# mcan1999/vulkan-raytracing

Hardware: AMD Instinct MI355X
Metric: Mrays/sec (primary+secondary) at 1920×1080 depth 4; 1/2/4/8-GPU scaling (higher is better)
Workload: dtype f32

## Files before the change

include/rt_api.h:

```cpp
#ifndef RT_API_H
#define RT_API_H

#include <stddef.h>
#include <stdint.h>

#ifdef __cplusplus
extern "C" {
#endif

typedef struct rt_ctx rt_ctx;

enum rt_status {
  RT_OK = 0,
  RT_ERR_INVALID_ARGUMENT = 1,
  RT_ERR_NOT_READY = 2,
  RT_ERR_DEVICE = 3,
  RT_ERR_OUT_OF_MEMORY = 4,
  RT_ERR_NO_DEVICE = 5
};

typedef struct rt_mesh_range {
  uint64_t first_float;
  uint64_t first_index;
  uint32_t prim_count;
// ... 86 lines not shown
#define RT_MATERIAL_TYPE_OF_INSTANCE 0xFFFFFFFFu
int rt_set_materials(rt_ctx* ctx, const rt_material* table, int n_materials, const uint32_t* prim_material, size_t n_prims);
int rt_set_instance_types(rt_ctx* ctx, const uint32_t* types, int n);

int rt_set_uniforms(rt_ctx* ctx, const rt_uniforms* u);

int rt_set_skybox(rt_ctx* ctx, const uint8_t* const faces_rgba8[6], int w, int h);

int rt_trace(rt_ctx* ctx, int width, int height, float* out_rgba32f_host, rt_stats* stats);

int rt_trace_shard(rt_ctx* ctx, int width, int height, int band_rows, int shard, int n_shards,
                   void* d_out, size_t out_capacity_bytes, void* hip_stream);
int rt_set_batch(rt_ctx* ctx, int n_frames, const rt_instance* instances, int n, const rt_uniforms* uniforms, int update);
int rt_trace_shard_batch(rt_ctx* ctx, int width, int height, int band_rows, int shard, int n_shards,
                         void* d_out, size_t frame_stride_bytes, size_t out_capacity_bytes, void* hip_stream);
int rt_trace_async(rt_ctx* ctx, int width, int height);
int rt_trace_wait(rt_ctx* ctx, const void** pixels, rt_stats* stats);

int rt_assemble_shards(rt_ctx* ctx, const void* d_gathered, int n_shards, size_t shard_stride_bytes, int width, int height,
                       int band_rows, void* d_frame, size_t frame_capacity_bytes, void* hip_stream);

int rt_shard_rows(int height, int band_rows, int shard, int n_shards);

int rt_synchronize(rt_ctx* ctx);
int rt_get_stats(rt_ctx* ctx, rt_stats* stats);
int rt_set_timing(rt_ctx* ctx, int enabled);

int rt_set_param(rt_ctx* ctx, const char* name, int value);

int rt_intersect(rt_ctx* ctx, size_t n, const float* rays8_host, int any_hit, rt_hit* out_host, int counting,
                 rt_stats* stats);

typedef struct rt_hit_attr {
  float position[3];
  int32_t object_index;
  float normal[3];
  uint32_t reserved;
} rt_hit_attr;

int rt_intersect_device(rt_ctx* ctx, size_t n, const void* d_rays8, int any_hit, void* d_hits, void* d_attr, void* hip_stream);

#define RT_RAY_FLAG_OPAQUE                 0x001u
#define RT_RAY_FLAG_NO_OPAQUE              0x002u
#define RT_RAY_FLAG_TERMINATE_ON_FIRST_HIT 0x004u
#define RT_RAY_FLAG_SKIP_CLOSEST_HIT       0x008u
#define RT_RAY_FLAG_CULL_BACK_FACING       0x010u
#define RT_RAY_FLAG_CULL_FRONT_FACING      0x020u
#define RT_RAY_FLAG_CULL_OPAQUE            0x040u
#define RT_RAY_FLAG_CULL_NO_OPAQUE         0x080u
#define RT_RAY_FLAG_SKIP_TRIANGLES         0x100u
#define RT_RAY_FLAG_SKIP_AABBS             0x200u
#define RT_INSTANCE_FLAG_FACING_CULL_DISABLE 0x1u
#define RT_INSTANCE_FLAG_FLIP_FACING         0x2u
#define RT_INSTANCE_FLAG_FORCE_OPAQUE        0x4u
#define RT_INSTANCE_FLAG_FORCE_NO_OPAQUE     0x8u
#define RT_HIT_KIND_FRONT_FACING 0xFEu
#define RT_HIT_KIND_BACK_FACING  0xFFu

int rt_intersect_device_flags(rt_ctx* ctx, size_t n, const void* d_rays8, const void* d_ray_words, uint32_t ray_flags, uint32_t cull_mask, void* d_hits, void* d_attr, void* hip_stream);

int rt_intersect_device_hits(rt_ctx* ctx, size_t n, const void* d_rays8, const void* d_ray_words, uint32_t ray_flags, uint32_t cull_mask,
                             uint32_t max_hits, void* d_hits, void* d_attr, void* d_counts, void* hip_stream);

int rt_closest_point_device(rt_ctx* ctx, size_t n, const void* d_points4, uint32_t cull_mask, void* d_hits, void* d_attr, void* hip_stream);
int rt_closest_point(rt_ctx* ctx, size_t n, const float* points4_host, uint32_t cull_mask, rt_hit* out_host, int counting, rt_stats* stats);

#define RT_OVERLAP_ANY 0x1u
int rt_overlap_boxes_device(rt_ctx* ctx, size_t n, const void* d_boxes8, uint32_t cull_mask, uint32_t flags,
                            uint32_t max_ids, void* d_ids, void* d_counts, void* hip_stream);
int rt_overlap_boxes(rt_ctx* ctx, size_t n, const float* boxes8_host, uint32_t cull_mask, uint32_t flags,
                     uint32_t max_ids, int32_t* ids_host, uint32_t* counts_host, int counting, rt_stats* stats);

int rt_sweep_spheres_device(rt_ctx* ctx, size_t n, const void* d_sweeps8, uint32_t cull_mask,
                            void* d_hits, void* d_attr, void* hip_stream);
int rt_sweep_spheres(rt_ctx* ctx, size_t n, const float* sweeps8_host, uint32_t cull_mask,
                     rt_hit* out_host, int counting, rt_stats* stats);

int rt_shade_rays_device(rt_ctx* ctx, size_t n_points, uint32_t n_samples, const void* d_rays8, void* d_sample_rgba, void* d_point_rgba, void* hip_stream);

int rt_trace_counting(rt_ctx* ctx, int width, int height, float* out_rgba32f_host, rt_stats* stats);

int rt_debug_check_builders(const float* verts6, size_t n_floats, const uint32_t* idx, size_t n_idx, uint64_t* out8);
int rt_debug_sizing(int n_cu, int resident_per_cu, int trace_blocks, uint32_t ovf_stride, uint64_t* out2);

const char* rt_last_error(const rt_ctx* ctx);
const char* rt_device_info(const rt_ctx* ctx);
int rt_abi_version(void);

#ifdef __cplusplus
}
#endif
#endif
```

vulkan_raytracing_amd/api.py:

```python
import ctypes as C

import numpy as np

from . import _native

HIT_DTYPE = np.dtype([("t", np.float32), ("u", np.float32), ("v", np.float32), ("prim", np.int32), ("inst", np.int32)])
MESH_RANGE_DTYPE = np.dtype([("first_float", np.uint64), ("first_index", np.uint64), ("prim_count", np.uint32), ("reserved", np.uint32)])
INSTANCE_DTYPE = np.dtype([("transform", np.float32, 12), ("custom_index_and_mask", np.uint32), ("sbt_offset_and_flags", np.uint32), ("mesh", np.uint64)])
UNIFORMS_DTYPE = np.dtype([("position", np.float32, 4), ("right", np.float32, 4), ("up", np.float32, 4), ("forward", np.float32, 4),
                           ("light_position", np.float32, 3), ("light_intensity", np.float32),
                           ("max_bounce_count", np.uint32), ("samples_per_pixel", np.uint32),
                           ("center_object_type", np.uint32), ("orbiting_object_type", np.uint32),
                           ("orbiting_object_primitive_offset", np.uint32), ("orbiting_object_vertex_offset", np.uint32)])
MATERIAL_DTYPE = np.dtype([("ka", np.float32, 3), ("ns", np.float32), ("kd", np.float32, 3), ("ni", np.float32), ("ks", np.float32, 3), ("type", np.uint32)])
MATERIAL_TYPE_OF_INSTANCE = 0xFFFFFFFF
assert MATERIAL_DTYPE.itemsize == 48
assert INSTANCE_DTYPE.itemsize == 64 and UNIFORMS_DTYPE.itemsize == 104 and MESH_RANGE_DTYPE.itemsize == 24


class RtStats(C.Structure):
    _fields_ = [("rays_primary", C.c_uint64), ("rays_secondary", C.c_uint64), ("rays_shadow", C.c_uint64),
                ("node_visits", C.c_uint64), ("tri_tests", C.c_uint64), ("node_visits_shadow", C.c_uint64), ("tri_tests_shadow", C.c_uint64),
                ("diag", C.c_uint64 * 6), ("closest_rays", C.c_uint64),
                ("ms_frame", C.c_float), ("ms_raygen", C.c_float), ("ms_trace_closest", C.c_float), ("ms_trace_shadow", C.c_float),
                ("ms_shade", C.c_float), ("ms_resolve", C.c_float),
                ("launches_trace_closest", C.c_uint32), ("launches_total", C.c_uint32), ("timed_frames", C.c_uint32), ("ms_tail", C.c_float),
                ("bvh_node_bytes", C.c_uint32), ("bvh_tri_bytes", C.c_uint32), ("tail_faults", C.c_uint32), ("frames_rerendered", C.c_uint32),
                ("blob_tiles", C.c_uint64), ("blob_tiles_large", C.c_uint64), ("blob_tiles_refused", C.c_uint64), ("blob_nodes", C.c_uint64), ("blob_tris", C.c_uint64),
                ("tile_rays", C.c_uint64), ("tile_rays_handed_on", C.c_uint64), ("tile_diag", C.c_uint64 * 6), ("rays_shadow_untraced", C.c_uint64)]

    def as_dict(self):
        return {k: (list(getattr(self, k)) if k in ("diag", "tile_diag") else getattr(self, k)) for k, _ in self._fields_}

    @property
    def rays_total(self):
        return self.rays_primary + self.rays_secondary + self.rays_shadow


RAY_FLAG_NONE = 0x000
RAY_FLAG_OPAQUE = 0x001
RAY_FLAG_NO_OPAQUE = 0x002
RAY_FLAG_TERMINATE_ON_FIRST_HIT = 0x004
RAY_FLAG_SKIP_CLOSEST_HIT = 0x008
RAY_FLAG_CULL_BACK_FACING = 0x010
RAY_FLAG_CULL_FRONT_FACING = 0x020
RAY_FLAG_CULL_OPAQUE = 0x040
RAY_FLAG_CULL_NO_OPAQUE = 0x080
RAY_FLAG_SKIP_TRIANGLES = 0x100
RAY_FLAG_SKIP_AABBS = 0x200
INSTANCE_FLAG_FACING_CULL_DISABLE = 0x1
INSTANCE_FLAG_FLIP_FACING = 0x2
INSTANCE_FLAG_FORCE_OPAQUE = 0x4
INSTANCE_FLAG_FORCE_NO_OPAQUE = 0x8
HIT_KIND_FRONT_FACING = 0xFE
HIT_KIND_BACK_FACING = 0xFF
OVERLAP_ANY = 0x1

EXPORTS = ["rt_create", "rt_create_frame_slot", "rt_destroy", "rt_upload_geometry", "rt_build_blas", "rt_set_instances", "rt_set_instances_device", "rt_refit_blas_device", "rt_set_materials", "rt_set_instance_types", "rt_set_uniforms", "rt_set_skybox",
           "rt_trace", "rt_trace_async", "rt_trace_wait", "rt_trace_shard", "rt_set_batch", "rt_trace_shard_batch", "rt_assemble_shards", "rt_shard_rows", "rt_synchronize", "rt_get_stats", "rt_set_timing", "rt_intersect",
           "rt_trace_counting", "rt_intersect_device", "rt_intersect_device_flags", "rt_intersect_device_hits", "rt_closest_point_device", "rt_closest_point", "rt_overlap_boxes_device", "rt_overlap_boxes", "rt_sweep_spheres_device", "rt_sweep_spheres", "rt_shade_rays_device", "rt_set_param", "rt_debug_check_builders", "rt_debug_sizing", "rt_last_error", "rt_device_info", "rt_abi_version"]

_LIBS = {}


def lib(variant=None):
    if variant not in _LIBS:
        L = _native.load_rt(variant)
        vp = C.c_void_p
        L.rt_create.argtypes = [C.POINTER(vp), C.c_int]
        L.rt_create_frame_slot.argtypes = [vp, C.POINTER(vp)]
        L.rt_destroy.argtypes = [vp]
        L.rt_destroy.restype = None
        L.rt_upload_geometry.argtypes = [vp, vp, C.c_size_t, vp, C.c_size_t, vp, C.c_int]
        L.rt_build_blas.argtypes = [vp, C.c_int]
        L.rt_set_instances.argtypes = [vp, vp, C.c_int, C.c_int]
        L.rt_set_instances_device.argtypes = [vp, vp, C.c_int, C.c_int, vp]
        L.rt_refit_blas_device.argtypes = [vp, C.c_int, vp, C.c_size_t, vp]
        L.rt_set_materials.argtypes = [vp, vp, C.c_int, vp, C.c_size_t]
        L.rt_set_instance_types.argtypes = [vp, vp, C.c_int]
        L.rt_set_uniforms.argtypes = [vp, vp]
        L.rt_set_skybox.argtypes = [vp, C.POINTER(vp), C.c_int, C.c_int]
        L.rt_trace.argtypes = [vp, C.c_int, C.c_int, vp, C.POINTER(RtStats)]
        L.rt_trace_counting.argtypes = [vp, C.c_int, C.c_int, vp, C.POINTER(RtStats)]
        L.rt_trace_async.argtypes = [vp, C.c_int, C.c_int]
        L.rt_trace_wait.argtypes = [vp, C.POINTER(vp), C.POINTER(RtStats)]
        L.rt_trace_shard.argtypes = [vp, C.c_int, C.c_int, C.c_int, C.c_int, C.c_int, vp, C.c_size_t, vp]
        L.rt_trace_shard_batch.argtypes = [vp, C.c_int, C.c_int, C.c_int, C.c_int, C.c_int, vp, C.c_size_t, C.c_size_t, vp]
        L.rt_set_batch.argtypes = [vp, C.c_int, vp, C.c_int, vp, C.c_int]
        L.rt_assemble_shards.argtypes = [vp, vp, C.c_int, C.c_size_t, C.c_int, C.c_int, C.c_int, vp, C.c_size_t, vp]
        L.rt_shard_rows.argtypes = [C.c_int] * 4
        L.rt_synchronize.argtypes = [vp]
        L.rt_get_stats.argtypes = [vp, C.POINTER(RtStats)]
        L.rt_set_timing.argtypes = [vp, C.c_int]
        L.rt_set_param.argtypes = [vp, C.c_char_p, C.c_int]
        L.rt_debug_check_builders.argtypes = [vp, C.c_size_t, vp, C.c_size_t, vp]
        L.rt_debug_sizing.argtypes = [C.c_int, C.c_int, C.c_int, C.c_uint32, vp]
        L.rt_intersect.argtypes = [vp, C.c_size_t, vp, C.c_int, vp, C.c_int, C.POINTER(RtStats)]
        L.rt_intersect_device.argtypes = [vp, C.c_size_t, vp, C.c_int, vp, vp, vp]
        L.rt_intersect_device_flags.argtypes = [vp, C.c_size_t, vp, vp, C.c_uint32, C.c_uint32, vp, vp, vp]
        L.rt_intersect_device_hits.argtypes = [vp, C.c_size_t, vp, vp, C.c_uint32, C.c_uint32, C.c_uint32, vp, vp, vp, vp]
        L.rt_closest_point_device.argtypes = [vp, C.c_size_t, vp, C.c_uint32, vp, vp, vp]
        L.rt_closest_point.argtypes = [vp, C.c_size_t, vp, C.c_uint32, vp, C.c_int, C.POINTER(RtStats)]
        L.rt_sweep_spheres_device.argtypes = [vp, C.c_size_t, vp, C.c_uint32, vp, vp, vp]
        L.rt_sweep_spheres.argtypes = [vp, C.c_size_t, vp, C.c_uint32, vp, C.c_int, C.POINTER(RtStats)]
        L.rt_overlap_boxes_device.argtypes = [vp, C.c_size_t, vp, C.c_uint32, C.c_uint32, C.c_uint32, vp, vp, vp]
        L.rt_overlap_boxes.argtypes = [vp, C.c_size_t, vp, C.c_uint32, C.c_uint32, C.c_uint32, vp, vp, C.c_int, C.POINTER(RtStats)]
        L.rt_shade_rays_device.argtypes = [vp, C.c_size_t, C.c_uint32, vp, vp, vp, vp]
        L.rt_last_error.argtypes = [vp]
        L.rt_last_error.restype = C.c_char_p
        L.rt_device_info.argtypes = [vp]
        L.rt_device_info.restype = C.c_char_p
        _LIBS[variant] = L
    return _LIBS[variant]


class RtError(RuntimeError):

    def __init__(self, code, fn, detail):
        super().__init__("RT API exception: return code %d (%s): %s" % (code, fn, detail))
        self.code = code


def _p(a):
    return a.ctypes.data_as(C.c_void_p)


class RtContext:

    def __init__(self, device=0, _parent=None, variant=None):
        self.L = _parent.L if _parent is not None else lib(variant)
        h = C.c_void_p()
        if _parent is not None:
            rc = self.L.rt_create_frame_slot(_parent.h, C.byref(h))
        else:
            rc = self.L.rt_create(C.byref(h), device)
        if rc:
            raise RtError(rc, "rt_create_frame_slot" if _parent is not None else "rt_create", self.L.rt_last_error(None).decode())
        self.h = h
        self.device = _parent.device if _parent is not None else device

    def frame_slot(self):
        return RtContext(_parent=self)

    def _chk(self, rc, fn):
        if rc:
            raise RtError(rc, fn, self.L.rt_last_error(self.h).decode())

    def close(self):
        if getattr(self, "h", None):
            self.L.rt_destroy(self.h)
            self.h = None

    def __del__(self):
        try:
            self.close()
        except Exception:
            pass

    @property
    def device_info(self):
        return self.L.rt_device_info(self.h).decode()

    def upload_geometry(self, verts6, idx, ranges, build=True):
        verts6 = np.ascontiguousarray(verts6, np.float32)
        idx = np.ascontiguousarray(idx, np.uint32)
        r = np.zeros(len(ranges), MESH_RANGE_DTYPE)
        for i, (ff, fi, pc) in enumerate(ranges):
            r[i] = (ff, fi, pc, 0)
        self._chk(self.L.rt_upload_geometry(self.h, _p(verts6), verts6.size, _p(idx), idx.size, _p(r), len(ranges)), "rt_upload_geometry")
        if build:
            for m in range(len(ranges)):
                self.build_blas(m)

    def build_blas(self, mesh):
        self._chk(self.L.rt_build_blas(self.h, mesh), "rt_build_blas")

    def set_instances(self, instances, update=False):
        inst = np.ascontiguousarray(instances, INSTANCE_DTYPE)
        self._chk(self.L.rt_set_instances(self.h, _p(inst), len(inst), int(update)), "rt_set_instances")
# ... 436 lines not shown
```

vulkan_raytracing_amd/csrc/kernels.hip:

```cpp
#include <hip/hip_runtime.h>

#include "rt_kernels.h"

namespace rt {

struct F3 { float x, y, z; };
__device__ __forceinline__ F3 mk3(float x, float y, float z) { F3 r; r.x = x; r.y = y; r.z = z; return r; }
__device__ __forceinline__ F3 add3(F3 a, F3 b) { return mk3(a.x + b.x, a.y + b.y, a.z + b.z); }
__device__ __forceinline__ F3 sub3(F3 a, F3 b) { return mk3(a.x - b.x, a.y - b.y, a.z - b.z); }
__device__ __forceinline__ F3 mul3(F3 a, float s) { return mk3(a.x * s, a.y * s, a.z * s); }
__device__ __forceinline__ F3 neg3(F3 a) { return mk3(-a.x, -a.y, -a.z); }
__device__ __forceinline__ float dot3(F3 a, F3 b) { return __builtin_fmaf(a.z, b.z, __builtin_fmaf(a.y, b.y, a.x * b.x)); }
__device__ __forceinline__ F3 cross3(F3 a, F3 b) {
  return mk3(__builtin_fmaf(a.y, b.z, -(a.z * b.y)), __builtin_fmaf(a.z, b.x, -(a.x * b.z)), __builtin_fmaf(a.x, b.y, -(a.y * b.x)));
}
__device__ __forceinline__ float length3(F3 v) { return __builtin_sqrtf(dot3(v, v)); }
__device__ __forceinline__ F3 normalize3(F3 v) { float inv = 1.0f / length3(v); return mul3(v, inv); }
__device__ __forceinline__ F3 fma3(float s, F3 a, F3 b) { return mk3(__builtin_fmaf(s, a.x, b.x), __builtin_fmaf(s, a.y, b.y), __builtin_fmaf(s, a.z, b.z)); }
__device__ __forceinline__ F3 reflect3(F3 I, F3 N) { float k = 2.0f * dot3(N, I); return fma3(-k, N, I); }

__device__ __forceinline__ F3 xform_point(const float* m, F3 p) {
  return mk3(__builtin_fmaf(m[2], p.z, __builtin_fmaf(m[1], p.y, m[0] * p.x)) + m[3],
             __builtin_fmaf(m[6], p.z, __builtin_fmaf(m[5], p.y, m[4] * p.x)) + m[7],
             __builtin_fmaf(m[10], p.z, __builtin_fmaf(m[9], p.y, m[8] * p.x)) + m[11]);
// ... 741 lines not shown
        for (uint32_t w = 0; w < blockDim.y; w++) { const float4 c = s_col[w][lane]; r += c.x; g += c.y; b += c.z; al += c.w; }
        const float nn = (float)spp;
        const uint32_t p = ly * (uint32_t)f.width + x;
        store_pixel(f, fi * f.out_frame_stride + p, make_float4(r / nn, g / nn, b / nn, al / nn));
        st_stream(&f.sample_color[fi * spp * npx1 + p], make_float4(0.f, 0.f, 0.f, PIXEL_DONE));
      }
    } else if (missed) st_stream(&f.sample_color[sid], miss_col);
  }
  if (survive || run_tile) {
    const uint32_t v = shard * f.shard_cap + slot;
    if (!f.pixel_runs) {
      const F3 o = f.batch_k > 1 ? mk3(bt.position[fi][0], bt.position[fi][1], bt.position[fi][2]) : mk3(u.position[0], u.position[1], u.position[2]);
      st_stream(&f.ray_o[0][v], make_float4(o.x, o.y, o.z, f.entry != nullptr ? __uint_as_float(tile) : 10000.0f));
    }
    st_stream(&f.ray_d[0][v], survive ? make_float4(d.x, d.y, d.z, __uint_as_float(sid)) : make_float4(0.f, 0.f, 0.f, __uint_as_float(SID_DEAD)));
  }
}

struct TraceArgs {
  SceneDev sc;
  const float4* ray_o;
  const float4* ray_d;
  const uint32_t* tails;
  uint32_t* work;
  uint32_t shard_cap;
  float4* hit_a;
  int32_t* hit_inst;
  const float4* sh_c;
  float4* sample_color;
  HitRec* raw_out;
  int32_t* ovf_stack;
  uint32_t* counters;
  union {
    float tmin;
    uint32_t query_word;
  };
  uint32_t rays_per_lane;
  uint32_t min_blocks;
  const EntryRec* entry;
  union {
    const uint32_t* sh_e;
    const uint32_t* ray_words;
  };
};

constexpr int MODE_CLOSEST = 0;
constexpr int MODE_SHADOW = 1;
constexpr int MODE_QUERY = 3;
constexpr int MODE_QUERY_FLAGS = 4;


#ifndef RT_REFILL_MIN
#define RT_REFILL_MIN 16
#endif
#ifndef RT_KEEP_NUM
#define RT_KEEP_NUM 5
#endif
#ifndef RT_INTERIOR_UNROLL
#define RT_INTERIOR_UNROLL 2
#endif
#ifndef RT_WIDE_UNROLL
#define RT_WIDE_UNROLL 1
#endif
#ifndef RT_WAVES_PER_EU
#define RT_WAVES_PER_EU 5
#endif
#ifndef RT_LEAF_CHAIN
#define RT_LEAF_CHAIN 1
#endif
#ifndef RT_STACK2_LDS
#define RT_STACK2_LDS 12
#endif
constexpr int STACK2_LDS = RT_STACK2_LDS;
constexpr uint32_t REFILL_MIN = RT_REFILL_MIN;

#ifdef RT_EXP_PHASE_SEL
#define PH_BEGIN(k) uint64_t ph_b##k = 0; if (COUNT && RT_EXP_PHASE_SEL == k) ph_b##k = __builtin_readcyclecounter();
#define PH_END(k) if (COUNT && RT_EXP_PHASE_SEL == k && lane == 0) { diag_iters++; diag_busy += __builtin_readcyclecounter() - ph_b##k; }
#else
#define PH_BEGIN(k)
#define PH_END(k)
#endif

template <int MODE, bool ANY, bool COUNT, bool WIDE, bool ENTRY = false, bool FAR = true, bool CONT = false>
__device__ __forceinline__ void trace_body(const TraceArgs& a) {
  constexpr bool RAYS8 = MODE == MODE_QUERY || MODE == MODE_QUERY_FLAGS;
  constexpr bool QF = MODE == MODE_QUERY_FLAGS;
  __shared__ int s_stack[4][STACK2_LDS + 1][64];
  __shared__ float4 s_rays[4][2][64];
  __shared__ float4 s_out[4][64];
  __shared__ int2 s_outq[4][64];
  __shared__ uint32_t s_ent[((ENTRY && MODE == MODE_SHADOW) || QF) ? 4 : 1][64];
  __shared__ float4 s_inst[LDS_INSTANCES ? LDS_INSTANCES : 1][5];
  {
    uint32_t total = 0;
#pragma unroll
    for (int t = 0; t < N_SHARDS; t++) total += ld_cursor(a.tails + t * CNT_STRIDE);
    uint32_t want = (total + 256u * a.rays_per_lane - 1u) / (256u * a.rays_per_lane);
    want = (want + (N_SHARDS - 1)) & ~(uint32_t)(N_SHARDS - 1);
    if (want < a.min_blocks) want = a.min_blocks;
    if (blockIdx.x >= want) return;
  }
  const int n_lds_inst = a.sc.n_inst < LDS_INSTANCES ? a.sc.n_inst : LDS_INSTANCES;
  if ((int)threadIdx.x < n_lds_inst) {
    const InstanceDev* I = a.sc.inst + threadIdx.x;
    const float4* mp = reinterpret_cast<const float4*>(I->w2o);
    s_inst[threadIdx.x][0] = mp[0]; s_inst[threadIdx.x][1] = mp[1]; s_inst[threadIdx.x][2] = mp[2];
    s_inst[threadIdx.x][3] = make_float4(I->q_lo[0], I->q_lo[1], I->q_lo[2], __int_as_float(I->blas_root));
    s_inst[threadIdx.x][4] = make_float4(I->q_scale[0], I->q_scale[1], I->q_scale[2], __uint_as_float(I->mask));
  }
  __syncthreads();
  const uint32_t lane = threadIdx.x & 63u, wave = threadIdx.x >> 6;
  int* const stk = &s_stack[wave][0][lane];
  int32_t* const ovf = a.ovf_stack + (size_t)(blockIdx.x * 256u + threadIdx.x) * a.sc.ovf_stride;
  uint64_t cnt_nodes = 0, cnt_tris = 0, diag_iters = 0, diag_busy = 0;
  const uint64_t diag_t0 = COUNT ? __builtin_readcyclecounter() : 0;

  uint32_t shard = blockIdx.x & (N_SHARDS - 1), tried = 0;
  uint32_t pf_base = 0, pf_count = 0;
  float4 pf_o = make_float4(0, 0, 0, 0), pf_d = pf_o;
  uint32_t pf_e = ENTRY_FROM_ROOT;
  uint32_t chunk_base = 0, chunk_count = 0, chunk_pos = 0;
  auto prefetch = [&]() {
    pf_count = 0;
    while (tried < (uint32_t)N_SHARDS) {
      const uint32_t size = ld_cursor(a.tails + shard * CNT_STRIDE);
      uint32_t off = 0;
      if (lane == 0 && size) off = atomicAdd(a.work + shard * CNT_STRIDE, 64u);
      off = (uint32_t)__builtin_amdgcn_readfirstlane((int)off);
      if (size && off < size) { pf_base = shard * a.shard_cap + off; pf_count = (size - off) < 64u ? (size - off) : 64u; break; }
      shard = (shard + 1u) & (N_SHARDS - 1); tried++;
    }
    if (lane < pf_count) {
      if constexpr (RAYS8) {
        const size_t r = 2u * (size_t)(pf_base + lane);
        pf_o = ld_stream(&a.ray_o[r]); pf_d = ld_stream(&a.ray_o[r + 1u]);
        if (QF) {
          const uint32_t w = a.ray_words ? (uint32_t)ld_stream(reinterpret_cast<const int*>(a.ray_words) + pf_base + lane) : 0xFF000000u;
          pf_e = ((a.query_word | w) & QF_FLAGS) | (a.query_word & w & 0xFF000000u);
        }
      } else {
        pf_o = ld_stream(&a.ray_o[pf_base + lane]); pf_d = ld_stream(&a.ray_d[pf_base + lane]);
      }
      if (ENTRY && MODE == MODE_SHADOW) pf_e = (uint32_t)ld_stream(reinterpret_cast<const int*>(a.sh_e) + pf_base + lane);
    }
  };
  auto promote = [&]() {
    s_rays[wave][0][lane] = pf_o; s_rays[wave][1][lane] = pf_d;
    if ((ENTRY && MODE == MODE_SHADOW) || QF) s_ent[wave][lane] = pf_e;
    chunk_base = pf_base; chunk_count = pf_count; chunk_pos = 0;
    prefetch();
  };
  prefetch();
  promote();

  uint32_t out_count = 0;
  auto flush = [&]() {
    if (lane < out_count) {
      const float4 r = s_out[wave][lane];
      const int2 k = s_outq[wave][lane];
      if (MODE == MODE_CLOSEST) { st_stream(&a.hit_a[k.x], r); st_stream(&a.hit_inst[k.x], k.y); }
      else if (MODE == MODE_SHADOW) {
        float cr = 0.08f, cg = 0.24f, cb = 0.08f;
        if (r.x != 0.0f || a.sc.n_materials != 0) {
          const float4 shc = ld_stream(&a.sh_c[(uint32_t)k.y]);
          if (r.x != 0.0f) { cr = shc.x; cg = shc.y; cb = shc.z; }
          else { const F3 amb = ambient_of(a.sc, __float_as_uint(shc.w)); cr = amb.x; cg = amb.y; cb = amb.z; }
        }
        st_stream(&a.sample_color[(uint32_t)k.x], make_float4(cr, cg, cb, 1.0f));
      }
      else { HitRec h; h.t = r.x; h.u = r.y; h.v = r.z; h.prim = (int)__float_as_uint(r.w); h.inst = k.y; a.raw_out[k.x] = h; }
    }
    out_count = 0;
  };

  bool need = true;
  uint32_t q = 0, sid = 0;
  float tmin_ray = 0.f, tmax = 0.f;
  uint32_t qword = 0;
  F3 wo = mk3(0, 0, 0), wd = mk3(0, 0, 1), co = wo, cd = wd, qs = mk3(1, 1, 1), qb = mk3(0, 0, 0);
  uint3 rot = make_uint3(0u, 0u, 0u);
  bool far = false;
  float best_t = 0.f, best_u = 0.f, best_v = 0.f;
  int best_prim = -1, best_inst = -1, cur_inst = -1, sp = 0, cur = REF_DONE;
  const char* const node_bytes = WIDE ? reinterpret_cast<const char*>(a.sc.wide_nodes) : reinterpret_cast<const char*>(a.sc.blas_nodes);

  auto push = [&](int v) {
    if (sp < STACK2_LDS) stk[sp * 64] = v;
    else *reinterpret_cast<volatile int32_t*>(ovf + (sp - STACK2_LDS)) = v;
    sp++;
  };
  auto pop = [&]() {
    sp--;
    if (sp < STACK2_LDS) cur = stk[sp * 64];
    else cur = *reinterpret_cast<volatile int32_t*>(ovf + (sp - STACK2_LDS));
  };

  auto to_instance = [&](int ii, int& root, uint32_t& imask) {
    float4 m0, m1, m2, ql, qsc;
    if (ii < n_lds_inst) { m0 = s_inst[ii][0]; m1 = s_inst[ii][1]; m2 = s_inst[ii][2]; ql = s_inst[ii][3]; qsc = s_inst[ii][4]; }
    else {
      const InstanceDev* I = a.sc.inst + ii;
      const float4* mp = reinterpret_cast<const float4*>(I->w2o);
      m0 = mp[0]; m1 = mp[1]; m2 = mp[2];
      ql = make_float4(I->q_lo[0], I->q_lo[1], I->q_lo[2], __int_as_float(I->blas_root));
      qsc = make_float4(I->q_scale[0], I->q_scale[1], I->q_scale[2], __uint_as_float(I->mask));
    }
    root = __float_as_int(ql.w); imask = __float_as_uint(qsc.w);
    if ((imask & 0xFFu) != 0u) {
      float m[12];
      m[0] = m0.x; m[1] = m0.y; m[2] = m0.z; m[3] = m0.w; m[4] = m1.x; m[5] = m1.y; m[6] = m1.z; m[7] = m1.w;
      m[8] = m2.x; m[9] = m2.y; m[10] = m2.z; m[11] = m2.w;
      co = xform_point(m, wo); cd = xform_vec(m, wd);
      const float qlo3[3] = {ql.x, ql.y, ql.z}, qsc3[3] = {qsc.x, qsc.y, qsc.z};
      quant_space(co, cd, qlo3, qsc3, qs, qb, rot); far = FAR && quant_far_o(co, qlo3, qsc3);
    }
  };

  for (;;) {
    PH_BEGIN(5)
    const uint64_t need_mask = __ballot(need);
    const uint32_t n_need = (uint32_t)__builtin_popcountll(need_mask);
    if (n_need >= REFILL_MIN || n_need == 64u) {
      if (chunk_pos == chunk_count && pf_count > 0) promote();
      if (chunk_pos < chunk_count) {
        const uint32_t rank = prefix_rank(need_mask);
        const uint32_t avail = chunk_count - chunk_pos;
        if (need && rank < avail) {
          const uint32_t ci = chunk_pos + rank;
          q = chunk_base + ci;
          const float4 ro = s_rays[wave][0][ci], rd = s_rays[wave][1][ci];
          if (RAYS8) { tmin_ray = ro.w; tmax = rd.w; }
          else { tmax = ro.w; sid = __float_as_uint(rd.w); }
          if (QF) qword = s_ent[wave][ci];
          wo = mk3(ro.x, ro.y, ro.z); wd = mk3(rd.x, rd.y, rd.z);
          co = wo; cd = wd;
          cur_inst = -1;
          stk[0] = REF_DONE;
          bool handed_on = false;
          if (CONT && (__float_as_uint(ro.w) & CONT_FLAG) != 0u) {
            handed_on = true;
            const uint32_t ent = __float_as_uint(ro.w);
            const uint32_t tile = ent & 0xFFFFFFu, mask = (ent >> 24) & 15u;
            const int4* rp = reinterpret_cast<const int4*>(a.entry + tile);
            const int4 r0 = rp[0], r1 = rp[1];
            const uint32_t n_rest = (((uint32_t)r0.x >> 4) & 15u) - 1u;
            const int wk[4] = {r0.z, r0.w, r1.x, r1.y};
            sp = 1;
#pragma unroll
            for (uint32_t k = 0; k < 4u; k++)
              if (k < n_rest && ((mask >> (n_rest - 1u - k)) & 1u) != 0u) { stk[sp * 64] = wk[k]; sp++; }
            sp--; cur = stk[sp * 64];
            quant_space(co, cd, a.sc.tlas_q_lo, a.sc.tlas_q_scale, qs, qb, rot); far = false;
            const float4 inc = a.hit_a[q];
            best_t = inc.x; best_u = inc.y; best_v = inc.z; best_prim = (int)__float_as_uint(inc.w); best_inst = a.hit_inst[q];
          } else
          if (ENTRY) {
            uint32_t ent;
            if (MODE == MODE_SHADOW) ent = s_ent[wave][ci];
            else ent = __float_as_uint(ro.w);
            const bool rev_flag = MODE == MODE_SHADOW && (ent & ENTRY_REVERSE) != 0u;
            if (MODE == MODE_SHADOW) ent &= ~ENTRY_REVERSE;
            int4 r0 = make_int4((int)ENTRY_EMPTY, REF_DONE, 0, 0), r1 = make_int4(0, 0, 0, 0);
            if (ent != ENTRY_FROM_ROOT) {
              const int4* rp = reinterpret_cast<const int4*>(a.entry + ent);
              r0 = rp[0]; r1 = rp[1];
            }
            const uint32_t hdr = (uint32_t)r0.x;
            if (ent == ENTRY_FROM_ROOT) {
              quant_space(co, cd, a.sc.tlas_q_lo, a.sc.tlas_q_scale, qs, qb, rot); far = FAR && quant_far_o(co, a.sc.tlas_q_lo, a.sc.tlas_q_scale);
              sp = 1; cur = a.sc.tlas_root + (a.sc.batch_samples ? (int)frame_of(sid, a.sc.batch_samples) * a.sc.tlas_stride : 0);
            } else if (hdr == ENTRY_EMPTY) {
              sp = 1; cur = REF_DONE;
            } else {
              const uint32_t nw = hdr & 15u, n_rm = (hdr >> 4) & 15u, ia = hdr >> 8;
              const bool rev = MODE == MODE_SHADOW && rev_flag && nw > n_rm;
              int cur_new = r0.y;
              const int wk[6] = {r0.z, r0.w, r1.x, r1.y, r1.z, r1.w};
#pragma unroll
              for (uint32_t k = 0; k < 6u; k++)
                if (k < nw) {
                  if (rev && k == n_rm) cur_new = wk[k];
                  else stk[((!rev || k < n_rm) ? 1u + k : 1u + nw + n_rm - k) * 64u] = wk[k];
                }
              if (rev) stk[(1u + n_rm) * 64u] = r0.y;
              sp = 1 + (int)nw;
              cur = cur_new;
              __builtin_amdgcn_sched_barrier(0);
              if (ia != ENTRY_NO_INST) { int root; uint32_t imask; to_instance((int)ia, root, imask); cur_inst = (int)ia; }
              else { quant_space(co, cd, a.sc.tlas_q_lo, a.sc.tlas_q_scale, qs, qb, rot); far = FAR && quant_far_o(co, a.sc.tlas_q_lo, a.sc.tlas_q_scale); }
            }
          } else {
            quant_space(co, cd, a.sc.tlas_q_lo, a.sc.tlas_q_scale, qs, qb, rot); far = FAR && quant_far_o(co, a.sc.tlas_q_lo, a.sc.tlas_q_scale);
            sp = 1;
            cur = a.sc.tlas_root;
            if (!RAYS8 && a.sc.batch_samples) cur += (int)frame_of(sid, a.sc.batch_samples) * a.sc.tlas_stride;
          }
          if (!(CONT && handed_on)) { best_t = (ENTRY && MODE == MODE_CLOSEST) ? 10000.0f : tmax; best_u = 0.f; best_v = 0.f; best_prim = -1; best_inst = -1; }
          need = false;
        }
        chunk_pos += n_need < avail ? n_need : avail;
      } else if (n_need == 64u) { flush(); break; }
    }
    PH_END(5)
    const uint32_t live = 64u - (uint32_t)__builtin_popcountll(__ballot(need));
    const uint32_t keep_going = (live * RT_KEEP_NUM + 7u) >> 3;

    auto interior_step = [&]() {
      if (WIDE) {
        if (cur >= 0) {
          const uint4* np = reinterpret_cast<const uint4*>(node_bytes + ((uint32_t)cur << 6));
          const uint4 X = np[0], Y = np[1], Z = np[2], R = np[3];
          if (COUNT) cnt_nodes++;
// ... 314 lines not shown
          const F3 spec = mk3((Iv * ks.x) * sp, (Iv * ks.y) * sp, (Iv * ks.z) * sp);
          const F3 amb = ambient_of(a.sc, mat);
          sh_c = fma3(w, add3(diff, spec), amb); sh_w = __uint_as_float(mat);
          nd = L; sh_tmax = dist;
          push_shadow = true;
          if (f.settle_dead_shadow_rays && __float_as_uint(sh_c.x) == __float_as_uint(amb.x) && __float_as_uint(sh_c.y) == __float_as_uint(amb.y) &&
              __float_as_uint(sh_c.z) == __float_as_uint(amb.z)) {
            st_stream(&f.sample_color[sid], make_float4(amb.x, amb.y, amb.z, 1.0f));
            push_shadow = false; settled = true;
          }
          if (f.light_entry != nullptr) {
            const F3 v = sub3(no, light);
            const float ax = __builtin_fabsf(v.x), ay = __builtin_fabsf(v.y), az = __builtin_fabsf(v.z);
            const int axis = (ax >= ay && ax >= az) ? 0 : (ay >= az ? 1 : 2);
            const float vc = axis == 0 ? v.x : (axis == 1 ? v.y : v.z), va = axis == 0 ? v.y : (axis == 1 ? v.z : v.x), vb = axis == 0 ? v.z : (axis == 1 ? v.x : v.y);
            const float c = __builtin_fabsf(vc);
            if (c > 0.0f) {
              const float T8 = (float)(8 * f.light_tiles);
              const float px = (va / c + 1.0f) * 0.5f * T8, py = (1.0f - vb / c) * 0.5f * T8;
              const int tx = min(max((int)(px * 0.125f), 0), f.light_tiles - 1), ty = min(max((int)(py * 0.125f), 0), f.light_tiles - 1);
              const int face = 2 * axis + (vc < 0.0f ? 1 : 0);
              sh_ent = (uint32_t)((face * f.light_tiles + ty) * f.light_tiles + tx) | (NdotL < 0.0f ? ENTRY_REVERSE : 0u);
            }
          }
        }
      } else if (type == 1u) {
        no = fma3(0.01f, N, P);
        nd = reflect3(d, N);
        push_next = true;
      } else if (type == 2u) {
        float ndoti = dot3(d, N);
        const bool outwards = ndoti > 0.0f;
        if (outwards) { N = neg3(N); ndoti = -ndoti; }
        const float ratio = M ? (outwards ? M->ni : 1.0f / M->ni) : (outwards ? 1.52f : (1.0f / 1.52f));
        const float k = 1.0f - (ratio * ratio) * (1.0f - ndoti * ndoti);
        if (k < 0.0f) { nd = reflect3(d, N); no = fma3(0.01f, N, P); }
        else {
          const float c = __builtin_fmaf(ratio, ndoti, __builtin_sqrtf(k));
          nd = normalize3(fma3(-c, N, mul3(d, ratio)));
          no = fma3(-0.01f, N, P);
        }
        push_next = true;
      } else {
        if (bounce == 0 && f.pixel_runs) {
          no = mk3(U.position[0], U.position[1], U.position[2]);
          if constexpr (BATCH) { const uint32_t fk = frame_of(sid, a.sc.batch_samples); no = mk3(a.bt.position[fk][0], a.bt.position[fk][1], a.bt.position[fk][2]); }
        } else {
          const float4 ro = ld_stream(&f.ray_o[cur][q]);
          no = mk3(ro.x, ro.y, ro.z);
        }
        nd = d; push_next = true;
      }
      if (push_next && last) {
        push_next = false;
        st_stream(&f.sample_color[sid], ambient_default<REG>());
      }
    }
  }
  {
    const uint64_t m_st = __ballot(settled);
    if (lane == 0 && m_st != 0ull) {
      __hip_atomic_fetch_add(f.counters + cnt_tail(Q_SHADOW0, (int)shard), (uint32_t)__builtin_popcountll(m_st), __ATOMIC_RELAXED, __HIP_MEMORY_SCOPE_AGENT);
      __hip_atomic_fetch_add(f.counters + cnt_work(Q_DEAD, (int)shard), (uint32_t)__builtin_popcountll(m_st), __ATOMIC_RELAXED, __HIP_MEMORY_SCOPE_AGENT);
    }
  }
  const uint32_t slot_n = wave_alloc(push_next, f.counters + cnt_tail(bounce + 1, (int)shard));
  if (push_next) {
    const uint32_t v = shard * f.shard_cap + slot_n;
    st_stream(&f.ray_o[nxt][v], make_float4(no.x, no.y, no.z, 10000.0f));
    st_stream(&f.ray_d[nxt][v], make_float4(nd.x, nd.y, nd.z, __uint_as_float(sid)));
  }
  if constexpr (RUNS) {
    if (in_range) {
      if (push_shadow) {
        st_stream(&f.sh_o[q], make_float4(no.x, no.y, no.z, sh_tmax));
        st_stream(&f.sh_c[q], make_float4(sh_c.x, sh_c.y, sh_c.z, sh_w));
        if (f.sh_e != nullptr) f.sh_e[q] = sh_ent;
      }
      st_stream(&f.sh_d[q], push_shadow ? make_float4(nd.x, nd.y, nd.z, __uint_as_float(sid)) : make_float4(0.f, 0.f, 0.f, __uint_as_float(SID_DEAD)));
    }
    const uint64_t m_sh = __ballot(push_shadow);
    if (lane == 0 && m_sh != 0ull) __hip_atomic_fetch_add(f.counters + cnt_tail(Q_SHADOW0, (int)shard), (uint32_t)__builtin_popcountll(m_sh), __ATOMIC_RELAXED, __HIP_MEMORY_SCOPE_AGENT);
  } else {
    const uint32_t slot_s = wave_alloc(push_shadow, f.counters + cnt_tail(Q_SHADOW, (int)shard));
    if (push_shadow) {
      const uint32_t v = f.sh_base + shard * f.shard_cap + slot_s;
      st_stream(&f.sh_o[v], make_float4(no.x, no.y, no.z, sh_tmax));
      st_stream(&f.sh_d[v], make_float4(nd.x, nd.y, nd.z, __uint_as_float(sid)));
      st_stream(&f.sh_c[v], make_float4(sh_c.x, sh_c.y, sh_c.z, sh_w));
      if (f.sh_e != nullptr) f.sh_e[v] = sh_ent;
    }
  }
}

template <bool TILE = false, bool BATCH = false, bool RUNS = false>
__device__ __forceinline__ void shade_body(const ShadeArgs& a, const int bounce) {
  const FrameDev& f = a.f;
  const UniformsDev& U = a.u;
  const uint32_t lane = threadIdx.x & 63u, wave = threadIdx.x >> 6;
  const int n_pass = TILE ? 2 : 1;
  for (int pass = 0; pass < n_pass; pass++) {
  uint32_t cnt[N_SHARDS], maxb = 0;
#pragma unroll
  for (int t = 0; t < N_SHARDS; t++) {
    if (TILE && pass) {
      uint32_t blobs = 0;
#pragma unroll
      for (int k = 0; k < BLOB_CLASSES; k++) blobs += ld_cursor(f.counters + cnt_tail(Q_BLOB_LIST + k, t));
      cnt[t] = blobs * (256u * ((U.samples_per_pixel + 3u) / 4u));
    } else cnt[t] = ld_cursor(f.counters + cnt_tail(bounce, t));
    maxb = max(maxb, (cnt[t] + 63u) >> 6);
  }
  const uint32_t n_waves = gridDim.x * 4u;
  for (uint32_t g = blockIdx.x * 4u + wave; g < maxb * N_SHARDS; g += n_waves) {
    const uint32_t shard = g & (N_SHARDS - 1), base = (g >> 3) << 6;
    uint32_t n = 0;
#pragma unroll
    for (int t = 0; t < N_SHARDS; t++) n = (shard == (uint32_t)t) ? cnt[t] : n;
    if (base >= n) continue;
    const uint32_t q = shard * f.shard_cap + ((TILE && pass) ? f.shard_cap - n : 0u) + base + lane;
    shade_slot<TILE, BATCH, RUNS, false>(a, bounce, shard, q, base + lane < n, HIT_DEAD, make_float4(0.f, 0.f, 0.f, 0.f));
  }
  }
}

template <bool TILE, bool BATCH, bool RUNS = false>
__global__ __launch_bounds__(256) void k_shade(ShadeArgs a) { shade_body<TILE, BATCH, RUNS>(a, a.bounce); }

#include "kernels_beam.inc"

struct TailArgs {
  TraceArgs tr;
  ShadeArgs sh;
  uint32_t first_bounce;
  uint32_t* barrier;
  uint32_t* fault;
};

__device__ __forceinline__ void grid_barrier(uint32_t* bar, uint32_t* fault, uint32_t& phase) {
  __syncthreads();
  phase++;
  if (threadIdx.x == 0) {
    __threadfence();
    const uint32_t target = phase * gridDim.x;
    __hip_atomic_fetch_add(bar, 1u, __ATOMIC_RELAXED, __HIP_MEMORY_SCOPE_AGENT);
    uint32_t spins = 0;
    while (__hip_atomic_load(bar, __ATOMIC_RELAXED, __HIP_MEMORY_SCOPE_AGENT) < target) {
      __builtin_amdgcn_s_sleep(8);
      if (++spins > (1u << 24)) { __hip_atomic_store(fault, 1u, __ATOMIC_RELAXED, __HIP_MEMORY_SCOPE_AGENT); break; }
    }
    __threadfence();
  }
  __syncthreads();
}

template <bool COUNT, bool WIDE, bool BATCH = false>
__global__ __launch_bounds__(256) void k_tail(TailArgs t) {
  uint32_t phase = 0;
  const uint32_t max_bounce = t.sh.u.max_bounce_count;
  for (uint32_t b = t.first_bounce; b <= max_bounce; b++) {
    uint32_t live = 0;
#pragma unroll
    for (int k = 0; k < N_SHARDS; k++) live += ld_cursor(t.tr.counters + cnt_tail((int)b, k));
    if (live == 0 || ld_cursor(t.fault) != 0u) break;
    TraceArgs a = t.tr;
    a.ray_o = t.sh.f.ray_o[b & 1u]; a.ray_d = t.sh.f.ray_d[b & 1u];
    a.tails = t.tr.counters + cnt_tail((int)b, 0);
    a.work = t.tr.counters + cnt_work((int)b, 0);
    trace_body<MODE_CLOSEST, false, COUNT, WIDE>(a);
    grid_barrier(t.barrier, t.fault, phase);
    if (ld_cursor(t.fault) != 0u) return;
    shade_body<false, BATCH>(t.sh, (int)b);
    grid_barrier(t.barrier, t.fault, phase);
    if (ld_cursor(t.fault) != 0u) return;
  }
}

__global__ __launch_bounds__(256) void k_resolve(FrameDev f, UniformsDev u) {
  const uint32_t npx1 = (uint32_t)(f.rows * f.width);
  const uint32_t lane = threadIdx.x & 63u, wave = (uint32_t)__builtin_amdgcn_readfirstlane((int)(threadIdx.x >> 6));
  const uint32_t tile_rows1 = ((uint32_t)f.rows + 7u) >> 3;
  const uint32_t trow = blockIdx.y * 4u + wave;
  if (trow < tile_rows1 * (uint32_t)f.batch_k) {
    const uint32_t fi = f.batch_k > 1 ? trow / tile_rows1 : 0u, by = trow - fi * tile_rows1;
    const uint32_t x = blockIdx.x * 8u + (lane & 7u), ly = by * 8u + (lane >> 3);
    if (!tile_is_sky(f, fi, blockIdx.x, by, trow * gridDim.x + blockIdx.x) && x < (uint32_t)f.width && ly < (uint32_t)f.rows) {
      const uint32_t p1 = ly * (uint32_t)f.width + x;
      const size_t s0 = (size_t)fi * u.samples_per_pixel * npx1 + p1;
      if (f.sample_color[s0].w != PIXEL_DONE) {
        float r = 0.f, g = 0.f, b = 0.f, al = 0.f;
        for (uint32_t i = 0; i < u.samples_per_pixel; i++) {
          const float4 c = ld_stream(&f.sample_color[s0 + (size_t)i * npx1]);
          r += c.x; g += c.y; b += c.z; al += c.w;
        }
        const float nn = (float)u.samples_per_pixel;
        store_pixel(f, fi * f.out_frame_stride + p1, make_float4(r / nn, g / nn, b / nn, al / nn));
      }
    }
  }
  const uint32_t p = (blockIdx.y * gridDim.x + blockIdx.x) * blockDim.x + threadIdx.x, n_threads = gridDim.x * gridDim.y * blockDim.x;
  if (f.counters_next)
    for (uint32_t i = p; i < (uint32_t)CNT_WORDS; i += n_threads) f.counters_next[i] = 0u;
  if (f.cover_next)
    for (uint32_t i = p; i < f.cover_words; i += n_threads) f.cover_next[i] = 0u;
  if (blockIdx.x == 0 && blockIdx.y == 0 && f.stats_out) {
    __shared__ unsigned long long s_q[N_QUEUES];
    const uint32_t t = threadIdx.x;
    if (t < (uint32_t)N_QUEUES) {
      unsigned long long n = 0;
      for (int k = 0; k < N_SHARDS; k++) n += ld_cursor(f.counters + cnt_tail((int)t, k));
      s_q[t] = n;
    }
    __syncthreads();
    if (f.hint && t >= 1u && t < (uint32_t)CNT_MAX_BOUNCES)
      __hip_atomic_store(f.hint + t, (uint32_t)(s_q[t] > 0xFFFFFFFFull ? 0xFFFFFFFFull : s_q[t]), __ATOMIC_RELAXED, __HIP_MEMORY_SCOPE_SYSTEM);
    auto cnt64 = [&](int word) { return (unsigned long long)ld_cursor(f.counters + word) | ((unsigned long long)ld_cursor(f.counters + word + 1) << 32); };
    if (t < (uint32_t)STAT_WORDS) {
      unsigned long long v = 0;
      if (t == STAT_QUEUE0) { v = s_q[0] + s_q[Q_TILE_RAYS] - s_q[Q_DEAD]; for (int k = 0; k < N_SHARDS; k++) v -= ld_cursor(f.counters + cnt_work(Q_TILE_RAYS, k)); }
      else if (t == STAT_TILE_RAYS) v = s_q[Q_TILE_RAYS];
      else if (t == STAT_CONT_RAYS) { for (int k = 0; k < N_SHARDS; k++) v += ld_cursor(f.counters + cnt_work(Q_TILE_RAYS, k)); }
      else if (t >= STAT_BLOB && t < STAT_BLOB + 5) v = ld_cursor(f.counters + CNT_BLOB_STATS + (int)(t - STAT_BLOB));
      else if (t >= STAT_TILE_DIAG && t < STAT_TILE_DIAG + 6) v = cnt64(CNT_TILE_DIAG + 2 * (int)(t - STAT_TILE_DIAG));
      else if (t == STAT_SECONDARY) { for (uint32_t b = 1; b <= u.max_bounce_count && b < (uint32_t)CNT_MAX_BOUNCES; b++) v += s_q[b]; }
      else if (t == STAT_SHADOW) v = s_q[Q_SHADOW] + s_q[Q_SHADOW0];
      else if (t == STAT_SHADOW_UNTRACED) { for (int k = 0; k < N_SHARDS; k++) v += ld_cursor(f.counters + cnt_work(Q_DEAD, k)); }
      else if (t == STAT_QUEUE1) v = s_q[1];
      else if (t == STAT_FAULT) v = ld_cursor(f.counters + CNT_FAULT);
      else if (t == STAT_FAULT_TOTAL) {
        uint32_t total = f.fault_total ? f.fault_total[0] : 0u;
        if (f.fault_total && ld_cursor(f.counters + CNT_FAULT) != 0u) { total++; f.fault_total[0] = total; }
        v = total;
      }
      else if (t == STAT_NODE_VISITS) v = cnt64(CNT_NODE_VISITS);
      else if (t == STAT_TRI_TESTS) v = cnt64(CNT_TRI_TESTS);
      else if (t == STAT_NODE_VISITS_SH) v = cnt64(CNT_NODE_VISITS_SH);
      else if (t == STAT_TRI_TESTS_SH) v = cnt64(CNT_TRI_TESTS_SH);
      else if (t >= STAT_DIAG && t < STAT_DIAG + 3) v = cnt64(CNT_DIAG + 2 * (int)(t - STAT_DIAG));
      else if (t >= STAT_DIAG + 3 && t < STAT_DIAG + 6) v = cnt64(CNT_DIAG_SH + 2 * (int)(t - STAT_DIAG - 3));
      __hip_atomic_store(f.stats_out + t, v, __ATOMIC_RELAXED, __HIP_MEMORY_SCOPE_SYSTEM);
    }
  }
}

int trace_threads_per_block() { return 256; }

static dim3 raygen_grid(int width, int rows, uint32_t spp, int batch_k, dim3& block) {
  const uint32_t wpb = spp < 4u ? spp : 4u;
  block = dim3(64, wpb);
  return dim3(((uint32_t)width + 7u) >> 3, (((uint32_t)rows + 7u) >> 3) * (uint32_t)batch_k, (spp + wpb - 1u) / wpb);
}
size_t raygen_block_count(int width, int rows, uint32_t spp, int batch_k) {
  dim3 b; const dim3 g = raygen_grid(width, rows, spp, batch_k, b);
  return (size_t)g.x * g.y * g.z;
}
void launch_raygen(const SceneDev& sc, const FrameDev& f, const UniformsDev& u, const BatchTab& bt, hipStream_t s) {
  dim3 b; const dim3 g = raygen_grid(f.width, f.rows, u.samples_per_pixel, f.batch_k, b);
  hipLaunchKernelGGL(k_raygen, g, b, 0, s, sc, f, u, bt);
}
size_t jitter_table_elems(int width, int rows, uint32_t spp) {
  return (size_t)(((uint32_t)width + 7u) >> 3) * (size_t)(((uint32_t)rows + 7u) >> 3) * spp * 64u;
}
void launch_jitter_table(const FrameDev& f, uint32_t spp, float2* table, hipStream_t s) {
  dim3 b; const dim3 g = raygen_grid(f.width, f.rows, spp, 1, b);
  hipLaunchKernelGGL(k_jitter_table, g, b, 0, s, f, spp, table);
}

void launch_cover(const SceneDev& sc, const CoverViews& a, uint32_t max_boxes_per_instance, uint32_t* mask_block, hipStream_t s) {
  if (a.n <= 0 || a.v[0].n_inst <= 0 || max_boxes_per_instance == 0) return;
  hipLaunchKernelGGL(k_cover, dim3((max_boxes_per_instance + 255u) / 256u, (unsigned)a.v[0].n_inst, (unsigned)a.n), dim3(256), 0, s, sc, a, mask_block);
}

static TraceArgs make_args(const SceneDev& sc, uint32_t* counters, int queue, uint32_t shard_cap, int32_t* ovf) {
  TraceArgs a{};
  a.sc = sc;
  a.tmin = 0.001f;
  a.counters = counters;
  a.tails = counters + cnt_tail(queue, 0);
  a.work = counters + cnt_work(queue, 0);
  a.shard_cap = shard_cap;
  a.ovf_stack = ovf;
  a.rays_per_lane = 4; a.min_blocks = 8;
  return a;
}

template <int MODE, bool ANY>
static void launch_trace(const TraceArgs& a_in, bool counting, const LaunchCfg& cfg, hipStream_t s) {
  TraceArgs a = a_in;
  a.rays_per_lane = (uint32_t)cfg.rays_per_lane; a.min_blocks = (uint32_t)cfg.min_blocks;
  const dim3 g(cfg.trace_blocks), b(256);
#ifdef RT_ALT_KERNELS
  if (cfg.variant == 2) {
    if (counting) hipLaunchKernelGGL((k_trace_count<MODE, ANY, true>), g, b, 0, s, a);
    else hipLaunchKernelGGL((k_trace<MODE, ANY, true>), g, b, 0, s, a);
    return;
  }
  if (cfg.variant == 1) {
    if (counting) hipLaunchKernelGGL((k_trace4<MODE, ANY, true>), g, b, 0, s, a);
    else hipLaunchKernelGGL((k_trace4<MODE, ANY, false>), g, b, 0, s, a);
    return;
  }
#endif
  if (counting) hipLaunchKernelGGL((k_trace_count<MODE, ANY, false>), g, b, 0, s, a);
  else if constexpr (MODE == MODE_QUERY) hipLaunchKernelGGL((k_trace<MODE, ANY, false, false, true>), g, b, 0, s, a);
  else if (cfg.far) hipLaunchKernelGGL((k_trace<MODE, ANY, false, false, true>), g, b, 0, s, a);
  else hipLaunchKernelGGL((k_trace<MODE, ANY, false, false, false>), g, b, 0, s, a);
}

// ... 246 lines not shown
    if (valid && tmax > 0.001f) {
      F3 qs, qb; uint3 rot;
      quant_space(o, d, sc.tlas_q_lo, sc.tlas_q_scale, qs, qb, rot);
      const bool far = quant_far(qs, qb);
      const uint4* rp = reinterpret_cast<const uint4*>(sc.blas_nodes + sc.tlas_root);
      const uint4 Q0 = rp[0], Q1 = rp[1];
      float tn;
      const bool h0 = far || slab_q(Q0.x, Q0.y, Q0.z, qs, qb, rot, 0.001f, tmax, tn);
      const bool h1 = (far || slab_q(Q0.w, Q1.x, Q1.y, qs, qb, rot, 0.001f, tmax, tn)) && Q1.w != Q1.z;
      const int c0 = (int)Q1.z, c1 = (int)Q1.w;
      survive = (h0 && c0 < 0) || (h1 && c1 < 0);
#pragma unroll
      for (int k = 0; k < 2; k++) {
        const int ch = k ? c1 : c0;
        if ((k ? h1 : h0) && ch >= 0 && !survive) {
          const uint4* np = reinterpret_cast<const uint4*>(sc.blas_nodes + ch);
          const uint4 N0 = np[0], N1 = np[1];
          survive = far || slab_q(N0.x, N0.y, N0.z, qs, qb, rot, 0.001f, tmax, tn) || slab_q(N0.w, N1.x, N1.y, qs, qb, rot, 0.001f, tmax, tn);
        }
      }
    }
    if (!survive) {
      float4 c = make_float4(0.f, 0.f, 0.f, 0.f);
      if (valid) { const F3 s = sample_sky(sc, mk3(d.x, d.y, -d.z)); c = make_float4(s.x, s.y, s.z, 1.0f); }
      st_stream(&f.sample_color[sid], c);
    }
  }
  __shared__ uint32_t s_run[5];
  const uint64_t smask = __ballot(survive);
  if (lane == 0) s_run[wave] = (uint32_t)__builtin_popcountll(smask);
  __syncthreads();
  const uint32_t shard = blockIdx.x & (N_SHARDS - 1);
  if (threadIdx.x == 0) {
    uint32_t tot = 0;
    for (uint32_t w = 0; w < 4u; w++) { const uint32_t c = s_run[w]; s_run[w] = tot; tot += c; }
    s_run[4] = tot ? atomicAdd(f.counters + cnt_tail(0, (int)shard), tot) : 0u;
  }
  __syncthreads();
  if (survive) {
    const uint32_t v = shard * f.shard_cap + s_run[4] + s_run[wave] + prefix_rank(smask);
    st_stream(&f.ray_o[0][v], make_float4(o.x, o.y, o.z, tmax));
    st_stream(&f.ray_d[0][v], make_float4(d.x, d.y, d.z, __uint_as_float(sid)));
  }
}

__global__ __launch_bounds__(256) void k_resolve_points(const float4* __restrict__ sample_color, float4* __restrict__ out, uint32_t n_points,
                                                        uint32_t n_samples) {
  const uint32_t p = blockIdx.x * 256u + threadIdx.x;
  if (p >= n_points) return;
  float r = 0.f, g = 0.f, b = 0.f, al = 0.f;
  for (uint32_t i = 0; i < n_samples; i++) {
    const float4 c = ld_stream(&sample_color[p + (size_t)i * n_points]);
    r += c.x; g += c.y; b += c.z; al += c.w;
  }
  const float nn = (float)n_samples;
  out[p] = make_float4(r / nn, g / nn, b / nn, al / nn);
}

uint32_t ray_ingest_block_count(uint32_t n) { return (n + 255u) / 256u; }
void launch_ray_ingest(const SceneDev& sc, const FrameDev& f, const float4* rays, uint32_t n, hipStream_t s) {
  hipLaunchKernelGGL(k_ray_ingest, dim3(ray_ingest_block_count(n)), dim3(256), 0, s, sc, f, rays, n);
}
void launch_resolve_points(const float4* sample_color, float4* out, uint32_t n_points, uint32_t n_samples, hipStream_t s) {
  hipLaunchKernelGGL(k_resolve_points, dim3((n_points + 255u) / 256u), dim3(256), 0, s, sample_color, out, n_points, n_samples);
}

#include "kernels_closest.inc"

#include "kernels_overlap.inc"

#include "kernels_sweep.inc"

int tail_blocks_per_cu() {
  int n = 1 << 30, v = 0;
  if (hipOccupancyMaxActiveBlocksPerMultiprocessor(&v, k_tail<false, false>, 256, 0) != hipSuccess) return 0;
  n = min(n, v);
  if (hipOccupancyMaxActiveBlocksPerMultiprocessor(&v, k_tail<true, false>, 256, 0) != hipSuccess) return 0;
  n = min(n, v);
#ifdef RT_ALT_KERNELS
  if (hipOccupancyMaxActiveBlocksPerMultiprocessor(&v, k_tail<false, true>, 256, 0) != hipSuccess) return 0;
  n = min(n, v);
  if (hipOccupancyMaxActiveBlocksPerMultiprocessor(&v, k_tail<true, true>, 256, 0) != hipSuccess) return 0;
  n = min(n, v);
#endif
  return n;
}

void launch_tail(const SceneDev& sc, const FrameDev& f, const UniformsDev& u, const BatchTab& bt, int first_bounce, bool counting, const LaunchCfg& cfg, int tail_blocks, hipStream_t s) {
  TailArgs t{};
  t.tr = make_args(sc, f.counters, first_bounce, f.shard_cap, f.ovf_stack);
  t.tr.hit_a = f.hit_a; t.tr.hit_inst = f.hit_inst;
  t.tr.rays_per_lane = 1u; t.tr.min_blocks = 8u;
  t.sh = ShadeArgs{sc, f, u, first_bounce, bt};
  t.first_bounce = (uint32_t)first_bounce;
  t.barrier = f.counters + CNT_BARRIER; t.fault = f.counters + CNT_FAULT;
  const dim3 g((unsigned)tail_blocks), b(256);
#ifdef RT_ALT_KERNELS
  if (cfg.variant == 2) {
    if (counting) hipLaunchKernelGGL((k_tail<true, true>), g, b, 0, s, t);
    else hipLaunchKernelGGL((k_tail<false, true>), g, b, 0, s, t);
    return;
  }
#endif
  if (f.batch_k > 1) {
    if (counting) hipLaunchKernelGGL((k_tail<true, false, true>), g, b, 0, s, t);
    else hipLaunchKernelGGL((k_tail<false, false, true>), g, b, 0, s, t);
    return;
  }
  if (counting) hipLaunchKernelGGL((k_tail<true, false>), g, b, 0, s, t);
  else hipLaunchKernelGGL((k_tail<false, false>), g, b, 0, s, t);
}

void launch_shade(const SceneDev& sc, const FrameDev& f, const UniformsDev& u, const BatchTab& bt, int bounce, const LaunchCfg& cfg, hipStream_t s) {
  ShadeArgs a{sc, f, u, bounce, bt};
  if (f.batch_k > 1) hipLaunchKernelGGL((k_shade<false, true>), dim3(cfg.shade_blocks), dim3(256), 0, s, a);
#ifdef RT_ALT_KERNELS
  else if (bounce == 0 && f.shadow_runs) hipLaunchKernelGGL((k_shade<false, false, true>), dim3(cfg.shade_blocks), dim3(256), 0, s, a);
  else if (bounce == 0 && f.tile_blob != nullptr) hipLaunchKernelGGL((k_shade<true, false>), dim3(cfg.shade_blocks), dim3(256), 0, s, a);
#endif
  else hipLaunchKernelGGL((k_shade<false, false>), dim3(cfg.shade_blocks), dim3(256), 0, s, a);
}

template <typename T>
__global__ __launch_bounds__(256) void k_assemble(const T* __restrict__ gathered, T* __restrict__ out, uint32_t width, uint32_t height,
                                                   uint32_t band_rows, uint32_t n_shards, size_t shard_stride) {
  const uint32_t x = blockIdx.x * blockDim.x + threadIdx.x, y = blockIdx.y;
  if (x >= width || y >= height) return;
  const uint32_t band = y / band_rows, within = y - band * band_rows;
  const uint32_t shard = band % n_shards, local = (band / n_shards) * band_rows + within;
  out[(size_t)y * width + x] = gathered[(size_t)shard * shard_stride + (size_t)local * width + x];
}

void launch_assemble(const void* gathered, void* out, int width, int height, int band_rows, int n_shards, size_t shard_stride_px, bool rgba8, hipStream_t s) {
  const dim3 g(((uint32_t)width + 255u) / 256u, (uint32_t)height), b(256);
  if (rgba8) hipLaunchKernelGGL((k_assemble<uint32_t>), g, b, 0, s, (const uint32_t*)gathered, (uint32_t*)out, (uint32_t)width, (uint32_t)height, (uint32_t)band_rows, (uint32_t)n_shards, shard_stride_px);
  else hipLaunchKernelGGL((k_assemble<float4>), g, b, 0, s, (const float4*)gathered, (float4*)out, (uint32_t)width, (uint32_t)height, (uint32_t)band_rows, (uint32_t)n_shards, shard_stride_px);
}

void launch_resolve(const FrameDev& f, const UniformsDev& u, hipStream_t s) {
  const uint32_t tile_rows = (((uint32_t)f.rows + 7u) >> 3) * (uint32_t)f.batch_k;
  hipLaunchKernelGGL(k_resolve, dim3(((uint32_t)f.width + 7u) >> 3, (tile_rows + 3u) / 4u), dim3(256), 0, s, f, u);
}

}
```

vulkan_raytracing_amd/csrc/rt_api.cpp:

```cpp
#include "../../include/rt_api.h"

#include <hip/hip_runtime.h>

#include <algorithm>
#include <cmath>
#include <cstdio>
#include <cstring>
#include <map>
#include <mutex>
#include <queue>
#include <string>
#include <vector>

#include "blas_refit.h"
#include "bvh_build.h"
#include "bvh_gpu.h"
#include "rt_device.h"
#include "rt_kernels.h"
#include "tlas_gpu.h"

using namespace rt;

static_assert(sizeof(rt_instance) == 64, "rt_instance must mirror VkAccelerationStructureInstanceKHR (64 B)");
static_assert(sizeof(rt_uniforms) == 104, "rt_uniforms must mirror UniformStructure (104 B)");
static_assert(sizeof(rt_uniforms) == sizeof(UniformsDev), "uniform mirrors out of sync");
static_assert(sizeof(rt_hit) == sizeof(HitRec), "hit mirrors out of sync");
static_assert(sizeof(rt_mesh_range) == 24, "rt_mesh_range layout");
static_assert(sizeof(rt_material) == sizeof(MaterialDev), "material mirrors out of sync");
static_assert(sizeof(rt_hit_attr) == 2 * sizeof(float4), "rt_hit_attr is the two float4 k_hit_attr writes");

namespace {

thread_local std::string g_create_error;

std::mutex g_live_mutex;
std::map<int, int> g_live_slots;
int live_slots_on(int device) { std::lock_guard<std::mutex> lk(g_live_mutex); auto it = g_live_slots.find(device); return it == g_live_slots.end() ? 0 : it->second; }
void live_slots_add(int device, int d) { std::lock_guard<std::mutex> lk(g_live_mutex); g_live_slots[device] += d; }

struct Mesh {
  rt_mesh_range range{};
  bool built = false;
  bool gpu_built = false;
  Aabb bounds{};
  BuiltBvh bvh;
  Bvh4 bvh4;
  std::vector<BvhNodeQ> qnodes;
  float q_lo[3] = {0, 0, 0}, q_scale[3] = {1, 1, 1};
  std::vector<TriPacket> tris;
  int levels = 0;
  int32_t node_base = 0, node_base4 = 0;
  int32_t root = 0;
  uint32_t tri_base = 0;
  uint32_t cover_first = 0, cover_count = 0;
  uint32_t laid_count = 0;
  uint32_t span_floats = 0;
  int span_shared_with = -1;
  bool refitted = false;
  bool verts_on_device = false;
  bool poisoned = false;
  bool parents_ready = false;
};

struct TimedSpan { int cat; hipEvent_t a, b; };
enum { CAT_RAYGEN = 0, CAT_TRACE, CAT_SHADE, CAT_SHADOW, CAT_RESOLVE, CAT_FRAME, CAT_TAIL, CAT_N };

}

constexpr int MAX_SLOTS = 16;
struct JitterTable {
  int W = 0, H = 0, rows = 0, band_rows = 0, shard = 0, n_shards = 0; uint32_t spp = 0;
  float2* d = nullptr;
  hipEvent_t ready = nullptr;
  uint64_t last_use = 0;
};
constexpr size_t MAX_JITTER_TABLES = 8;

struct Scene {
  int device = 0;
  std::vector<rt_ctx*> members;
  uint32_t slot_mask = 0;
  std::vector<JitterTable> jitter_tables;
  uint64_t jitter_clock = 0;

  std::vector<float> h_verts;
  std::vector<uint32_t> h_idx;
  float* d_verts = nullptr;
  uint32_t* d_idx = nullptr;
  std::vector<Mesh> meshes;
  bool blas_linked = false;
  std::vector<BvhNodeQ> h_blasq;
  BvhNodeQ* d_blas_nodes = nullptr;
  std::vector<Bvh4Node> h_blas4;
  Bvh4Node* d_nodes4 = nullptr;
  std::vector<WideNodeQ> h_wide;
  WideNodeQ* d_wide = nullptr;
  float4* d_tris = nullptr;
  size_t n_blas_nodes = 0, n_blas4 = 0, n_tris = 0;
  float* d_cover_boxes = nullptr;
  uint32_t max_cover_count = 0;
  uint32_t tlas_cap = 1024;
  bool arrays_ready = false;
  int variant = 0;

  uchar4* d_sky = nullptr;
  int sky_w = 0, sky_h = 0;

  MaterialDev* d_materials = nullptr;
  uint32_t* d_prim_material = nullptr;
  int n_materials = 0;
  size_t n_prim_material = 0;

  TlasMeshDev* d_mesh_table = nullptr;
  uint32_t* d_cover_src = nullptr;
  BlasRefitScratch refit;
};

enum { INST_NONE = 0, INST_HOST = 1, INST_DEVICE = 2 };
constexpr int MAX_DEVICE_INSTANCES = 1 << 20;

struct rt_ctx {
  int device = 0;
  hipStream_t stream = nullptr;
  std::string error;
  std::string info;
  int n_cu = 0;
  Scene* scene = nullptr;
  int slot = 0;

  std::vector<rt_instance> h_inst;
  std::vector<uint32_t> inst_types;
  BuiltBvh tlas;
  Bvh4 tlas4;
  bool tlas_valid = false;
  bool tlas_stale = false;
  int inst_source = INST_NONE;
  int n_inst = 0;
  TlasGpu tgpu;
  bool dev_far = true;
  double dev_g_lo[3] = {0, 0, 0}, dev_g_hi[3] = {0, 0, 0};
  InstanceDev* d_inst[2] = {nullptr, nullptr};
  size_t cap_inst[2] = {0, 0};
  int parity = 0;
  int tlas_node_count[2] = {0, 0};
  int batch_k = 1;
  uint32_t batch_out_stride = 0;
  int inst_per_frame = 0;
  int tlas_stride[2] = {0, 0};
  std::vector<UniformsDev> batch_uni;
  hipEvent_t ev_frame[2] = {nullptr, nullptr};
  bool ev_frame_valid[2] = {false, false};
  float tlas_q_lo[3] = {0, 0, 0}, tlas_q_scale[3] = {1, 1, 1};
  uint32_t ovf_stride = STACK_OVF, ovf_alloc_stride = 0;
  int stack_need = 0;
  int ovf_alloc_blocks = 0;
  char* h_stage[2] = {nullptr, nullptr};
  size_t stage_bytes[2] = {0, 0};
  hipEvent_t ev_upload[2] = {nullptr, nullptr};
  bool upload_inflight[2] = {false, false};
  bool upload_pending = false;

  UniformsDev uni{};
  bool have_uni = false;

  FrameDev frame{};
  size_t frame_capacity = 0;
  size_t out_capacity = 0;
  float4* d_out_own = nullptr;
  float4* h_out_pinned = nullptr;
  size_t pinned_capacity = 0;
  bool out_rgba8 = false;
  bool out_bgra = false;
  bool async_pending = false;
  int async_w = 0, async_h = 0;
  uint32_t* d_counters = nullptr;
  int cnt_parity = 0;
  int32_t* d_ovf = nullptr;
  LaunchCfg cfg{};
  bool grid_user_set = false;
  int closest_blocks_per_cu = -1, shadow_blocks_per_cu = -1;
  int tail_blocks = TAIL_BLOCKS;
  int tail_resident_per_cu = 0;
  int tail_mode = 1;
  int jitter_table = 1;
  const float2* jitter_waited = nullptr; hipStream_t jitter_waited_stream = nullptr;
  int primary_cover = 1;
  int tail_min_blocks = 1;
  bool tail_full_grid = false;
  int entry_max_instances = 32;
  int entry_points = 1;
  int shadow_entry = 2;
  int light_tiles = LIGHT_TILES_DEFAULT;
  EntryRec* d_entry = nullptr;
  size_t entry_alloc_tiles = 0;
  int camera_records = 1;
  int dead_shadow_rays = 1;
  int shadow_beams = 0;
  bool sh_double = false;
  int fused_shade = 1;
  int pixel_beams = 1;
  int tile_blobs = 0;
  uint32_t* d_tile_blob = nullptr;
  char* d_blob_arena = nullptr;
  uint32_t blob_slots = 0;
  uint4* d_blob_list = nullptr;
  size_t tile_dir_alloc = 0;
  EntryRec* d_light_entry = nullptr;
  size_t light_alloc_tiles = 0;
  uint32_t* d_cover_mask = nullptr;
  uint32_t cover_alloc_words = 0;
  int cover_parity = 0;
  unsigned long long* h_stats = nullptr;
  unsigned long long* d_stats = nullptr;
  bool last_empty = false;
  uint32_t* h_hint = nullptr;
  uint32_t* d_hint = nullptr;
  int blas_builder = 1;
  int timing = 0;
  bool counting = false;
  std::vector<hipEvent_t> ev_pool;
  size_t ev_used = 0;
  std::vector<TimedSpan> spans;
  uint32_t timed_frames = 0;
  rt_stats last{};
  bool frame_pending = false;
  hipStream_t frame_stream = nullptr;
  struct LastFrame { int W, H, band_rows, shard, n_shards; float4* d_out; bool counting; SceneDev sc; UniformsDev uni; int parity; uint64_t inst_gen; int batch_k; BatchTab bt; uint32_t out_frame_stride; } last_frame{};
  uint64_t inst_gen[2] = {0, 0};
  struct LightKey {
    float light[3] = {0, 0, 0}; uint64_t gen = 0; int parity = -1, n_inst = 0, tiles = 0;
    bool operator==(const LightKey& o) const { return light[0] == o.light[0] && light[1] == o.light[1] && light[2] == o.light[2] && gen == o.gen && parity == o.parity && n_inst == o.n_inst && tiles == o.tiles; }
  };
  LightKey light_key_seen, light_key_built;
  bool light_built = false, light_seen_valid = false;
  bool tail_disabled = false;
  bool frame_rerendered = false;
  uint32_t tail_faults = 0;
  uint32_t* d_fault_total = nullptr;
  uint64_t faults_seen = 0;
  bool debug_force_tail_fault = false;
  uint32_t last_max_bounce = 0;
  uint64_t last_primary = 0;
  uint32_t* d_q_counters = nullptr;
  int32_t* d_q_ovf = nullptr;
  size_t q_ovf_alloc = 0;
  float* d_q_scale = nullptr;
  size_t q_scale_alloc = 0;
  hipEvent_t ev_query[2] = {nullptr, nullptr};
  bool ev_query_valid[2] = {false, false};
  int query_last = -1;
  FrameDev shade{};
  size_t shade_capacity = 0;
  size_t shade_colors = 0;
};

namespace {

int fail(rt_ctx* c, int code, const std::string& msg) {
  if (c) c->error = msg; else g_create_error = msg;
  return code;
}
#define HIP_TRY(c, expr)                                                                          \
  do {                                                                                            \
    hipError_t e_ = (expr);                                                                       \
    if (e_ != hipSuccess)                                                                         \
      return fail(c, e_ == hipErrorOutOfMemory ? RT_ERR_OUT_OF_MEMORY : RT_ERR_DEVICE,            \
                  std::string("HIP runtime exception: return code ") + std::to_string((int)e_) +  \
                      " (" + hipGetErrorString(e_) + ") in " #expr);                              \
  } while (0)

void invert_affine(const float m[12], float out[12]) {
  double a = m[0], b = m[1], c = m[2], d = m[4], e = m[5], f = m[6], g = m[8], h = m[9], i = m[10];
  double tx = m[3], ty = m[7], tz = m[11];
  double c00 = e * i - f * h, c01 = c * h - b * i, c02 = b * f - c * e;
  double c10 = f * g - d * i, c11 = a * i - c * g, c12 = c * d - a * f;
  double c20 = d * h - e * g, c21 = b * g - a * h, c22 = a * e - b * d;
  double det = a * c00 + b * c10 + c * c20;
  double r = 1.0 / det;
  double n[9] = {c00 * r, c01 * r, c02 * r, c10 * r, c11 * r, c12 * r, c20 * r, c21 * r, c22 * r};
  out[0] = (float)n[0]; out[1] = (float)n[1]; out[2] = (float)n[2];
  out[4] = (float)n[3]; out[5] = (float)n[4]; out[6] = (float)n[5];
  out[8] = (float)n[6]; out[9] = (float)n[7]; out[10] = (float)n[8];
  out[3] = (float)(-(n[0] * tx + n[1] * ty + n[2] * tz));
  out[7] = (float)(-(n[3] * tx + n[4] * ty + n[5] * tz));
  out[11] = (float)(-(n[6] * tx + n[7] * ty + n[8] * tz));
}

Aabb instance_world_box(const float o2w[12], const Aabb& b) {
  Aabb w; for (int k = 0; k < 3; k++) { w.lo[k] = 3.0e38f; w.hi[k] = -3.0e38f; }
  if (b.lo[0] > b.hi[0]) { for (int k = 0; k < 3; k++) w.lo[k] = w.hi[k] = 3.0e38f; return w; }
  float mag = 0.f;
  for (int cx = 0; cx < 8; cx++) {
    double p[3] = {(cx & 1) ? b.hi[0] : b.lo[0], (cx & 2) ? b.hi[1] : b.lo[1], (cx & 4) ? b.hi[2] : b.lo[2]};
    for (int r = 0; r < 3; r++) {
      double v = o2w[4 * r] * p[0] + o2w[4 * r + 1] * p[1] + o2w[4 * r + 2] * p[2] + o2w[4 * r + 3];
      w.lo[r] = std::min(w.lo[r], (float)v); w.hi[r] = std::max(w.hi[r], (float)v);
      mag = std::max(mag, (float)std::fabs(v));
    }
  }
  float pad = 1e-5f * mag + 1e-30f;
  for (int k = 0; k < 3; k++) { w.lo[k] -= pad; w.hi[k] += pad; }
  return w;
}

}

size_t rt::ovf_elems(int trace_blocks, int tail_blocks, uint32_t stride) {
  return (size_t)std::max(trace_blocks, tail_blocks) * 256u * (size_t)stride;
}
int rt::tail_grid(int n_cu, int resident_blocks_per_cu, int live_slots) {
  const long cap = (long)n_cu * std::max(0, resident_blocks_per_cu) / std::max(MAX_TAILS_IN_FLIGHT, live_slots);
  long g = std::min<long>(TAIL_BLOCKS, cap);
  g -= g % N_SHARDS;
  return g >= N_SHARDS ? (int)g : 0;
}

namespace {

int alloc_scene_arrays(rt_ctx* c);
int wait_queries(rt_ctx* c, rt_ctx* m, int parity = -1);

static std::vector<BvhNodeQ> treelet_layout(const std::vector<BvhNodeQ>& in) {
  if (in.size() < 4) return in;
  std::vector<BvhNodeQ> out;
  out.reserve(in.size() + 8);
  std::vector<int32_t> new_of(in.size(), -1);
  std::vector<int32_t> todo;
  std::vector<int32_t> singles;
  size_t singles_at = 0;
  auto place = [&](int32_t old) { new_of[old] = (int32_t)out.size(); out.push_back(in[old]); };
  todo.push_back(0);
  while (!todo.empty()) {
    const int32_t r = todo.back(); todo.pop_back();
    const BvhNodeQ& q = in[r];
    int32_t kids[2]; int nk = 0;
    if (q.child0 >= 0) kids[nk++] = q.child0;
    if (q.child1 >= 0 && q.child1 != q.child0) kids[nk++] = q.child1;
    const size_t size = 1 + (size_t)nk;
    if (size == 1 && r != 0) {
      if (out.size() & 3u) place(r); else singles.push_back(r);
      continue;
    }
    if ((out.size() & 3u) + size > 4u)
      while (out.size() & 3u) { if (singles_at < singles.size()) place(singles[singles_at++]); else out.push_back(in[0]); }
    place(r);
    for (int k = 0; k < nk; k++) place(kids[k]);
    for (int k = nk - 1; k >= 0; k--) {
      const BvhNodeQ& c = in[kids[k]];
      if (c.child1 >= 0 && c.child1 != c.child0) todo.push_back(c.child1);
      if (c.child0 >= 0) todo.push_back(c.child0);
    }
  }
  while (singles_at < singles.size()) place(singles[singles_at++]);
  for (BvhNodeQ& q : out) {
    if (q.child0 >= 0) q.child0 = new_of[q.child0];
    if (q.child1 >= 0) q.child1 = new_of[q.child1];
  }
  return out;
}

int refit_mesh(rt_ctx* c, int mi, const float* src, hipStream_t src_stream);

int link_blas(rt_ctx* c) {
  Scene* S = c->scene;
  size_t nn = 0, nt = 0, nn4 = 0;
  static const bool line_layout = [] { const char* e = getenv("RT_NODE_LAYOUT"); return e ? atoi(e) != 0 : true; }();
  std::vector<std::vector<BvhNodeQ>> laid(S->meshes.size());
  std::vector<size_t> gap_from(S->meshes.size(), 0);
  for (size_t mi = 0; mi < S->meshes.size(); mi++) {
    Mesh& m = S->meshes[mi];
    if (!m.built) continue;
    if (!m.gpu_built) quantize_bvh2(m.bvh, m.qnodes, m.q_lo, m.q_scale);
    laid[mi] = line_layout ? treelet_layout(m.qnodes) : m.qnodes;
    if (getenv("RT_BUILD_TIMING")) fprintf(stderr, "[link_blas] mesh %zu: %zu nodes, %zu slots in the cache-line layout\n", mi, m.qnodes.size(), laid[mi].size());
    gap_from[mi] = nn;
    nn = (nn + 3u) & ~(size_t)3u;
    m.node_base = (int32_t)nn; m.tri_base = (uint32_t)nt; m.node_base4 = (int32_t)nn4;
    m.laid_count = (uint32_t)laid[mi].size(); m.parents_ready = false;
    nn += laid[mi].size(); nt += m.tris.size(); nn4 += m.bvh4.nodes.size();
  }
  std::vector<BvhNodeQ> nodes(nn);
  std::vector<Bvh4Node> nodes4(nn4);
  std::vector<TriPacket> tris(nt);
  for (size_t mi = 0; mi < S->meshes.size(); mi++) {
    Mesh& m = S->meshes[mi];
    if (!m.built) continue;
    const std::vector<BvhNodeQ>& mq = laid[mi];
    for (size_t i = gap_from[mi]; i < (size_t)m.node_base; i++) nodes[i] = nodes[0];
    for (size_t i = 0; i < mq.size(); i++) {
      BvhNodeQ n = mq[i];
      auto fix = [&](int32_t ch) -> int32_t {
// ... 287 lines not shown
  }
  double smin = std::min({(double)c->tlas_q_scale[0], (double)c->tlas_q_scale[1], (double)c->tlas_q_scale[2]});
  for (int k = 0; k < 3; k++)
    if (std::max(std::fabs(c->tlas_q_lo[k] - lo[k]), std::fabs(c->tlas_q_lo[k] - hi[k])) > K * smin) return true;
  if (c->inst_source == INST_DEVICE) {
    for (int k = 0; k < 3; k++)
      if (!((double)u.position[k] >= c->dev_g_lo[k] && (double)u.position[k] <= c->dev_g_hi[k])) return true;
    return c->dev_far;
  }
  for (const rt_instance& in : c->h_inst) {
    const Mesh& m = S->meshes[in.mesh];
    if (!m.range.prim_count) continue;
    float w2o[12];
    invert_affine(in.transform, w2o);
    smin = std::min({(double)m.q_scale[0], (double)m.q_scale[1], (double)m.q_scale[2]});
    for (int cx = 0; cx < 8; cx++) {
      const double p[3] = {(cx & 1) ? hi[0] : lo[0], (cx & 2) ? hi[1] : lo[1], (cx & 4) ? hi[2] : lo[2]};
      for (int r = 0; r < 3; r++) {
        const double v = w2o[4 * r] * p[0] + w2o[4 * r + 1] * p[1] + w2o[4 * r + 2] * p[2] + w2o[4 * r + 3];
        if (!(std::fabs(m.q_lo[r] - v) <= K * smin)) return true;
      }
    }
  }
  return false;
}

int quiesce(rt_ctx* c) {
  if (c->async_pending) return fail(c, RT_ERR_NOT_READY, "a frame submitted with rt_trace_async is pending: call rt_trace_wait first");
  if (c->frame_pending) return collect_stats(c);
  return RT_OK;
}
int wait_queries(rt_ctx* c, rt_ctx* m, int parity) {
  const int p = parity < 0 ? m->query_last : parity;
  if (p < 0 || !m->ev_query_valid[p]) return RT_OK;
  HIP_TRY(c, hipEventSynchronize(m->ev_query[p]));
  m->ev_query_valid[p] = false;
  if (parity < 0 || p == m->query_last) { m->ev_query_valid[0] = m->ev_query_valid[1] = false; m->query_last = -1; }
  return RT_OK;
}
int quiesce_scene(rt_ctx* c) {
  for (rt_ctx* m : c->scene->members) {
    { int q = wait_queries(c, m); if (q) return q; }
    if (m->async_pending) return fail(c, RT_ERR_NOT_READY, "a frame slot of this scene has a frame pending (rt_trace_async): collect it with rt_trace_wait first");
    if (m->frame_pending) { int r = collect_stats(m); if (r) { if (m != c) c->error = m->error; return r; } }
    for (int k = 0; k < 2; k++)
      if (m->upload_inflight[k]) { HIP_TRY(c, hipEventSynchronize(m->ev_upload[k])); m->upload_inflight[k] = false; }
    m->upload_pending = false;
  }
  return RT_OK;
}
void invalidate_tlas(Scene* S) { for (rt_ctx* m : S->members) { m->tlas_valid = false; m->tlas_stale = false; } }

int ready_to_trace(rt_ctx* c, bool batch = false) {
  if (!c->scene->d_verts) return fail(c, RT_ERR_NOT_READY, "rt_upload_geometry has not been called");
  if (!c->tlas_valid) return fail(c, RT_ERR_NOT_READY, "rt_set_instances has not been called");
  if (c->tlas_stale) return fail(c, RT_ERR_NOT_READY, "a BLAS was refitted (rt_refit_blas_device) since the TLAS was set: update it with rt_set_instances, rt_set_instances_device or rt_set_batch first");
  if (!batch && c->batch_k != 1) return fail(c, RT_ERR_NOT_READY, "the context holds a frame batch (rt_set_batch): render it with rt_trace_shard_batch, or call rt_set_instances for a single frame");
  return RT_OK;
}

int ensure_common(rt_ctx* c) {
  if (!c->d_counters) {
    HIP_TRY(c, hipMalloc((void**)&c->d_counters, 2 * CNT_WORDS * sizeof(uint32_t)));
    HIP_TRY(c, hipMemsetAsync(c->d_counters, 0, 2 * CNT_WORDS * sizeof(uint32_t), c->stream));
    HIP_TRY(c, hipStreamSynchronize(c->stream));
    c->cnt_parity = 0;
  }
  if (!c->d_fault_total) {
    HIP_TRY(c, hipMalloc((void**)&c->d_fault_total, sizeof(uint32_t)));
    HIP_TRY(c, hipMemsetAsync(c->d_fault_total, 0, sizeof(uint32_t), c->stream));
    HIP_TRY(c, hipStreamSynchronize(c->stream));
    c->faults_seen = 0;
  }
  if (!c->h_hint) {
    HIP_TRY(c, hipHostMalloc((void**)&c->h_hint, CNT_MAX_BOUNCES * sizeof(uint32_t), hipHostMallocMapped));
    for (int b = 0; b < CNT_MAX_BOUNCES; b++) c->h_hint[b] = 0xFFFFFFFFu;
    HIP_TRY(c, hipHostGetDevicePointer((void**)&c->d_hint, c->h_hint, 0));
  }
  if (!c->h_stats) {
    HIP_TRY(c, hipHostMalloc((void**)&c->h_stats, STAT_WORDS * sizeof(unsigned long long), hipHostMallocMapped));
    memset(c->h_stats, 0, STAT_WORDS * sizeof(unsigned long long));
    HIP_TRY(c, hipHostGetDevicePointer((void**)&c->d_stats, c->h_stats, 0));
  }
  if (c->d_ovf && (c->ovf_alloc_stride < c->ovf_stride || c->ovf_alloc_blocks < std::max(c->cfg.trace_blocks, c->tail_blocks))) { HIP_TRY(c, hipFree(c->d_ovf)); c->d_ovf = nullptr; }
  if (!c->d_ovf) {
    HIP_TRY(c, hipMalloc((void**)&c->d_ovf, ovf_elems(c->cfg.trace_blocks, c->tail_blocks, c->ovf_stride) * sizeof(int32_t)));
    c->ovf_alloc_stride = c->ovf_stride; c->ovf_alloc_blocks = std::max(c->cfg.trace_blocks, c->tail_blocks);
  }
  return RT_OK;
}

int alloc_queues(rt_ctx* c, FrameDev& f, size_t capacity, size_t sh_cap, size_t colors) {
  void** ptrs[] = {(void**)&f.ray_o[0], (void**)&f.ray_o[1], (void**)&f.ray_d[0], (void**)&f.ray_d[1], (void**)&f.hit_a};
  void** sh_ptrs[] = {(void**)&f.sh_o, (void**)&f.sh_d, (void**)&f.sh_c};
  for (void** p : ptrs) { if (*p) HIP_TRY(c, hipFree(*p)); *p = nullptr; }
  for (void** p : sh_ptrs) { if (*p) HIP_TRY(c, hipFree(*p)); *p = nullptr; }
  if (f.sample_color) { HIP_TRY(c, hipFree(f.sample_color)); f.sample_color = nullptr; }
  if (f.hit_inst) { HIP_TRY(c, hipFree(f.hit_inst)); f.hit_inst = nullptr; }
  if (f.sh_e) { HIP_TRY(c, hipFree(f.sh_e)); f.sh_e = nullptr; }
  for (void** p : ptrs) HIP_TRY(c, hipMalloc(p, capacity * sizeof(float4)));
  if (colors) HIP_TRY(c, hipMalloc((void**)&f.sample_color, colors * sizeof(float4)));
  for (void** p : sh_ptrs) HIP_TRY(c, hipMalloc(p, sh_cap * sizeof(float4)));
  HIP_TRY(c, hipMalloc((void**)&f.hit_inst, capacity * sizeof(int32_t)));
  HIP_TRY(c, hipMalloc((void**)&f.sh_e, sh_cap * sizeof(uint32_t)));
  return RT_OK;
}
void free_queues(FrameDev& f) {
  void* ptrs[] = {f.ray_o[0], f.ray_o[1], f.ray_d[0], f.ray_d[1], f.hit_a, f.hit_inst, f.sh_o, f.sh_d, f.sh_c, f.sh_e, f.sample_color};
  for (void* p : ptrs) if (p) hipFree(p);
}

int ensure_frame(rt_ctx* c, size_t capacity) {
  int r = ensure_common(c); if (r) return r;
  const bool want_double = c->shadow_beams != 0;
  if (capacity <= c->frame_capacity && (!want_double || c->sh_double)) return RT_OK;
  capacity = std::max(capacity, c->frame_capacity);
  c->frame_capacity = 0;
  const size_t sh_cap = (want_double ? 2 : 1) * capacity;
  r = alloc_queues(c, c->frame, capacity, sh_cap, capacity); if (r) return r;
  c->sh_double = want_double;
  c->frame_capacity = capacity;
  return RT_OK;
}

hipEvent_t take_event(rt_ctx* c) {
  if (c->ev_used == c->ev_pool.size()) { hipEvent_t e; hipEventCreate(&e); c->ev_pool.push_back(e); }
  return c->ev_pool[c->ev_used++];
}

int jitter_table_for(rt_ctx* c, const FrameDev& f, uint32_t spp, hipStream_t s, const float2** out) {
  Scene* S = c->scene;
  *out = nullptr;
  JitterTable* t = nullptr;
  for (JitterTable& k : S->jitter_tables)
    if (k.W == f.width && k.H == f.height && k.rows == f.rows && k.spp == spp && k.band_rows == f.band_rows && k.shard == f.shard && k.n_shards == f.n_shards) { t = &k; break; }
  if (!t) {
    if (S->jitter_tables.size() >= MAX_JITTER_TABLES) {
      HIP_TRY(c, hipDeviceSynchronize());
      size_t lru = 0;
      for (size_t k = 1; k < S->jitter_tables.size(); k++) if (S->jitter_tables[k].last_use < S->jitter_tables[lru].last_use) lru = k;
      hipFree(S->jitter_tables[lru].d); hipEventDestroy(S->jitter_tables[lru].ready);
      S->jitter_tables.erase(S->jitter_tables.begin() + (long)lru);
      for (rt_ctx* m : S->members) m->jitter_waited = nullptr;
    }
    JitterTable n;
    n.W = f.width; n.H = f.height; n.rows = f.rows; n.spp = spp; n.band_rows = f.band_rows; n.shard = f.shard; n.n_shards = f.n_shards;
    HIP_TRY(c, hipMalloc((void**)&n.d, jitter_table_elems(f.width, f.rows, spp) * sizeof(float2)));
    if (hipEventCreateWithFlags(&n.ready, hipEventDisableTiming) != hipSuccess) { hipFree(n.d); return fail(c, RT_ERR_DEVICE, "hipEventCreate failed"); }
    launch_jitter_table(f, spp, n.d, s);
    HIP_TRY(c, hipEventRecord(n.ready, s));
    S->jitter_tables.push_back(n);
    t = &S->jitter_tables.back();
    c->jitter_waited = t->d; c->jitter_waited_stream = s;
  }
  if (c->jitter_waited != t->d || c->jitter_waited_stream != s) {
    HIP_TRY(c, hipStreamWaitEvent(s, t->ready, 0));
    c->jitter_waited = t->d; c->jitter_waited_stream = s;
  }
  t->last_use = ++S->jitter_clock;
  *out = t->d;
  return RT_OK;
}

struct Span {
  rt_ctx* c; int cat; hipStream_t s; hipEvent_t a = nullptr;
  bool on() const { return c->timing == 1 || (c->timing == 2 && cat == CAT_TRACE); }
  Span(rt_ctx* c_, int cat_, hipStream_t s_) : c(c_), cat(cat_), s(s_) {
    if (on()) { a = take_event(c); hipEventRecord(a, s); }
  }
  ~Span() {
// ... 105 lines not shown
    f.entry = entry_on ? c->d_entry : nullptr;
    if (tile_on) {
      const uint32_t want_slots = (uint32_t)(((std::min<size_t>(tiles_local, tiles_local / 2 + 2048) + N_SHARDS - 1) / N_SHARDS + 8) * N_SHARDS);
      if (tiles_local > c->tile_dir_alloc || want_slots > c->blob_slots) {
        HIP_TRY(c, hipStreamSynchronize(c->stream)); if (s != c->stream) HIP_TRY(c, hipStreamSynchronize(s));
        if (c->d_tile_blob) HIP_TRY(c, hipFree(c->d_tile_blob));
        if (c->d_blob_arena) HIP_TRY(c, hipFree(c->d_blob_arena));
        if (c->d_blob_list) HIP_TRY(c, hipFree(c->d_blob_list));
        c->d_tile_blob = nullptr; c->d_blob_arena = nullptr; c->d_blob_list = nullptr; c->tile_dir_alloc = 0; c->blob_slots = 0;
        const size_t dir = std::max(tiles_local, c->entry_alloc_tiles);
        HIP_TRY(c, hipMalloc((void**)&c->d_tile_blob, dir * sizeof(uint32_t)));
        HIP_TRY(c, hipMalloc((void**)&c->d_blob_arena, (size_t)want_slots * BLOB_SLOT_BYTES));
        HIP_TRY(c, hipMalloc((void**)&c->d_blob_list, (size_t)BLOB_CLASSES * want_slots * sizeof(uint4)));
        c->tile_dir_alloc = dir; c->blob_slots = want_slots;
      }
      f.tile_blob = c->d_tile_blob; f.blob_arena = c->d_blob_arena; f.blob_slots = c->blob_slots; f.blob_list = c->d_blob_list;
    }
    if (entry_on)
      for (int fk = 0; fk < K; fk++) {
        EntryArgs& ea = ev.v[fk];
        const CoverArgs& cak = cv.v[fk];
        const float* right = K > 1 ? bt.right[fk] : u.right; const float* up = K > 1 ? bt.up[fk] : u.up; const float* fwd = K > 1 ? bt.forward[fk] : u.forward;
        for (int k = 0; k < 3; k++) ea.cam[k] = cak.cam[k];
        for (int k = 0; k < 9; k++) ea.inv[k] = cak.inv[k];
        for (int k = 0; k < 3; k++) { ea.basis[k] = right[k]; ea.basis[3 + k] = up[k]; ea.basis[6 + k] = fwd[k]; }
        ea.kf = 2.5f; ea.apex_radius = 0.0f;
        ea.width = W; ea.height = H; ea.tiles_x = (W + 7) / 8; ea.tile_rows = (rows + 7) / 8;
        ea.band_rows = band_rows; ea.shard = shard; ea.n_shards = n_shards;
        ea.records = c->d_entry + (size_t)fk * tiles_local; ea.cover = f.cover + (size_t)fk * cam_words; ea.cover_tiles_x = f.cover_tiles_x;
        ea.tlas_root_offset = fk * sc.tlas_stride;
      }
    ev.n = entry_on ? K : 1;
    if (light_on) {
      const size_t light_tiles_total = (size_t)6 * LT * LT;
      if (light_tiles_total > c->light_alloc_tiles) {
        if (c->d_light_entry) { HIP_TRY(c, hipStreamSynchronize(c->stream)); if (s != c->stream) HIP_TRY(c, hipStreamSynchronize(s)); HIP_TRY(c, hipFree(c->d_light_entry)); c->d_light_entry = nullptr; c->light_alloc_tiles = 0; }
        HIP_TRY(c, hipMalloc((void**)&c->d_light_entry, light_tiles_total * sizeof(EntryRec)));
        c->light_alloc_tiles = light_tiles_total; c->light_built = false;
      }
      f.light_entry = c->d_light_entry; f.light_tiles = LT;
      const float apex_radius = 0.0102f;
      for (int face = 0; face < 6; face++) {
        const int axis = face >> 1, a1 = (axis + 1) % 3, a2 = (axis + 2) % 3;
        const float sgn = (face & 1) ? -1.0f : 1.0f;
        float basis[9] = {0, 0, 0, 0, 0, 0, 0, 0, 0};
        basis[a1] = 1.0f; basis[3 + a2] = 1.0f; basis[6 + axis] = sgn;
        CoverArgs& lc = cv.v[1 + face];
        EntryArgs& le = ev.v[1 + face];
        for (int k = 0; k < 3; k++) lc.cam[k] = le.cam[k] = u.light_position[k];
        for (int k = 0; k < 9; k++) { lc.inv[k] = le.inv[k] = basis[k]; le.basis[k] = basis[k]; }
        lc.kf = le.kf = 1.0f; lc.apex_radius = le.apex_radius = apex_radius;
        lc.width = lc.height = le.width = le.height = 8 * LT;
        lc.tiles_x = lc.tiles_y = LT; lc.n_inst = ca.n_inst;
        lc.mask_offset = cam_words + (uint32_t)face * face_words;
        le.tiles_x = le.tile_rows = LT; le.band_rows = 8 * LT; le.shard = 0; le.n_shards = 1;
        le.records = c->d_light_entry + (size_t)face * LT * LT;
        le.cover = f.cover + lc.mask_offset; le.cover_tiles_x = LT;
      }
      bool build = true;
      if (c->shadow_entry == 2) {
        rt_ctx::LightKey key;
        for (int k = 0; k < 3; k++) key.light[k] = u.light_position[k];
        key.gen = c->inst_gen[frame_parity]; key.parity = frame_parity; key.n_inst = sc.n_inst; key.tiles = LT;
        const bool have = c->light_built && key == c->light_key_built;
        const bool stable = !c->light_seen_valid || key == c->light_key_seen;
        if (!again) { c->light_key_seen = key; c->light_seen_valid = true; }
        if (again != nullptr) { build = false; if (!have) { f.light_entry = nullptr; f.light_tiles = 0; } }
        else if (have) build = false;
        else if (stable) { c->light_key_built = key; c->light_built = true; }
        else { build = false; c->light_built = false; f.light_entry = nullptr; f.light_tiles = 0; }
      }
      if (build) { cv.n = ENTRY_VIEWS; ev.n = ENTRY_VIEWS; }
    }
  }
  LaunchCfg cfg = c->cfg;
  if (c->stack_need > 120) cfg.packet = 0;
  if (K > 1) cfg.packet = 0;
  cfg.far = far_frame ? 1 : 0;
  f.far_possible = cfg.far;
  f.settle_dead_shadow_rays = c->dead_shadow_rays;
  f.pixel_runs = beam_on ? 64 * (int)std::min<uint32_t>(u.samples_per_pixel, 4u) : 0;
  f.shadow_runs = (beam_on && c->shadow_beams && K == 1 && std::isfinite(u.light_position[0]) && std::isfinite(u.light_position[1]) && std::isfinite(u.light_position[2])) ? 1u : 0u;
  f.sh_base = f.shadow_runs ? (uint32_t)capacity : 0u;
  if (c->jitter_table && rows > 0) { r = jitter_table_for(c, f, u.samples_per_pixel, s, &f.jitter); if (r) return r; }
  if (!c->timing || c->timed_frames >= 64) { c->ev_used = 0; c->spans.clear(); c->timed_frames = 0; }
  if (c->timing) c->timed_frames++;
  c->frame_stream = s; c->frame_pending = true;
  c->last_max_bounce = u.max_bounce_count;
  c->last_primary = (uint64_t)W * rows * u.samples_per_pixel * (uint64_t)K;
  c->last_empty = rows == 0;
  if (c->upload_pending && s != c->stream) HIP_TRY(c, hipStreamWaitEvent(s, c->ev_upload[c->parity], 0));
  if (rows == 0) return RT_OK;
  c->cnt_parity ^= 1;
  if (f.cover_next) c->cover_parity ^= 1;
  int cap_closest = c->closest_blocks_per_cu, cap_shadow = c->shadow_blocks_per_cu;
  {
    constexpr unsigned long long GRID_SMALL_RAYS = 2500000ull;
    const bool crowded = c->scene->members.size() >= 3 && !c->grid_user_set && !c->last_empty;
    const unsigned long long prev_q0 = ((volatile unsigned long long*)c->h_stats)[STAT_QUEUE0], prev_sh = ((volatile unsigned long long*)c->h_stats)[STAT_SHADOW];
    if (cap_closest < 0) cap_closest = (crowded && prev_q0 > 0 && prev_q0 <= GRID_SMALL_RAYS) ? 2 : 0;
    if (cap_shadow < 0) cap_shadow = (crowded && f.light_entry != nullptr && prev_sh > 0 && prev_sh <= GRID_SMALL_RAYS) ? 2 : 0;
  }
  {
    Span frame_span(c, CAT_FRAME, s);
    {
      Span sp(c, CAT_RAYGEN, s);
      if (f.cover) launch_cover(sc, cv, c->scene->max_cover_count, const_cast<uint32_t*>(f.cover), s);
      if (f.entry || ev.n > 1) launch_entry(sc, ev, s);
      if (f.tile_blob) launch_blob(sc, ev.v[0], f, c->counting, s);
      launch_raygen(sc, f, u, bt, s);
    }
    uint32_t tail_start = 0xFFFFFFFFu;
    const bool tail_ok = c->cfg.variant != 1 && c->tail_blocks > 0 && !no_tail && !c->tail_disabled;
    if (tail_ok && c->tail_mode == 2) tail_start = 1;
    else if (tail_ok && c->tail_mode == 1)
      for (uint32_t b = 1; b <= u.max_bounce_count && b < (uint32_t)CNT_MAX_BOUNCES; b++)
        if (((volatile uint32_t*)c->h_hint)[b] <= TAIL_MAX_RAYS) { tail_start = b; break; }
    const bool fused0 = c->fused_shade && beam_on && c->camera_records && K == 1 && !c->counting && !f.tile_blob && !f.shadow_runs && tail_start != 0u;
    for (uint32_t b = 0; b <= u.max_bounce_count; b++) {
      if (b == tail_start) {
        int tb = std::min(c->tail_blocks, tail_grid(c->n_cu, c->tail_resident_per_cu, live_slots_on(c->device)));
        if (tb <= 0) { { Span sp(c, CAT_TRACE, s); launch_trace_closest(sc, f, (int)b, c->counting, cfg, s); } { Span sp(c, CAT_SHADE, s); launch_shade(sc, f, u, bt, (int)b, cfg, s); } continue; }
        const uint32_t expect = ((volatile uint32_t*)c->h_hint)[b];
        if (c->tail_mode == 1 && expect != 0xFFFFFFFFu && !c->tail_full_grid && c->scene->members.size() >= 3) {
          long want = ((long)expect + 255) / 256;
          const long lo = c->tail_min_blocks;
          if (lo >= N_SHARDS) want = (want + (N_SHARDS - 1)) / N_SHARDS * N_SHARDS;
          tb = (int)std::min<long>(tb, std::max<long>(lo, want));
        }
        Span sp(c, CAT_TAIL, s); launch_tail(sc, f, u, bt, (int)b, c->counting, cfg, tb, s);
        break;
      }
      { LaunchCfg cc = cfg; if (b == 0 && cap_closest > 0) cc.trace_blocks = std::min(cfg.trace_blocks, c->n_cu * cap_closest);
        Span sp(c, CAT_TRACE, s);
        if (b == 0 && f.tile_blob) launch_tile(sc, f, u, c->counting, s);
        if (b == 0 && fused0) launch_beam_shade(sc, f, u, cc, s);
        else launch_trace_closest(sc, f, (int)b, c->counting, cc, s); }
      if (!(b == 0 && fused0)) { Span sp(c, CAT_SHADE, s); launch_shade(sc, f, u, bt, (int)b, cfg, s); }
      if (b >= 7 && (b & 3) == 3 && b < u.max_bounce_count) {
        uint32_t tails[N_SHARDS * CNT_STRIDE];
        HIP_TRY(c, hipMemcpyAsync(tails, f.counters + cnt_tail((int)b + 1, 0), sizeof(tails), hipMemcpyDeviceToHost, s));
        HIP_TRY(c, hipStreamSynchronize(s));
        uint32_t live = 0;
        for (int t = 0; t < N_SHARDS; t++) live += tails[t * CNT_STRIDE];
        if (live == 0) break;
      }
    }
    { LaunchCfg cs = cfg; if (cap_shadow > 0) cs.trace_blocks = std::min(cfg.trace_blocks, c->n_cu * cap_shadow);
      Span sp(c, CAT_SHADOW, s); launch_beam_shadow(sc, f, u, c->counting, cs, s); launch_trace_shadow(sc, f, c->counting, cs, s); }
    { Span sp(c, CAT_RESOLVE, s); launch_resolve(f, u, s); }
  }
  HIP_TRY(c, hipGetLastError());
  if (!c->ev_frame[frame_parity]) HIP_TRY(c, hipEventCreateWithFlags(&c->ev_frame[frame_parity], hipEventDisableTiming));
  HIP_TRY(c, hipEventRecord(c->ev_frame[frame_parity], s));
  c->ev_frame_valid[frame_parity] = true;
  return RT_OK;
}

int collect_stats(rt_ctx* c) {
  if (!c->frame_pending) return RT_OK;
  HIP_TRY(c, hipStreamSynchronize(c->frame_stream));
  c->upload_pending = false;
  const unsigned long long* hs = c->h_stats;
  rt_stats st{};
  st.rays_primary = c->last_primary;
  if (!c->last_empty) {
    st.rays_secondary = hs[STAT_SECONDARY];
    st.rays_shadow = hs[STAT_SHADOW]; st.rays_shadow_untraced = hs[STAT_SHADOW_UNTRACED];
    const uint64_t total = hs[STAT_FAULT_TOTAL];
    const bool forced = c->debug_force_tail_fault && !c->tail_disabled;
    if (total != c->faults_seen || forced) {
      c->tail_faults += (uint32_t)(total - c->faults_seen) + ((forced && hs[STAT_FAULT] == 0) ? 1u : 0u);
      c->faults_seen = total;
      c->tail_disabled = true;
    }
    if (hs[STAT_FAULT] != 0 || forced) {
      c->debug_force_tail_fault = false;
      const rt_ctx::LastFrame lf = c->last_frame;
      if (c->inst_gen[lf.parity] != lf.inst_gen) {
        c->frame_pending = false;
        return fail(c, RT_ERR_DEVICE, "a k_tail grid barrier gave up and the frame cannot be rendered again: rt_set_instances replaced its instance records "
                                      "twice before the frame was collected (collect every frame, or update the instances at most once per frame)");
      }
      const bool counting = c->counting;
      c->counting = lf.counting;
      c->ev_used = 0; c->spans.clear(); c->timed_frames = 0;
      int r = enqueue_frame(c, lf.W, lf.H, lf.band_rows, lf.shard, lf.n_shards, lf.d_out, c->frame_stream, &lf);
      c->counting = counting;
      if (r) { c->frame_pending = false; return r; }
      c->frame_rerendered = true;
      return collect_stats(c);
    }
    st.closest_rays = hs[STAT_QUEUE0] + st.rays_secondary;
    st.node_visits = hs[STAT_NODE_VISITS]; st.tri_tests = hs[STAT_TRI_TESTS];
    st.node_visits_shadow = hs[STAT_NODE_VISITS_SH]; st.tri_tests_shadow = hs[STAT_TRI_TESTS_SH];
    for (int k = 0; k < 6; k++) st.diag[k] = hs[STAT_DIAG + k];
    st.blob_tiles = hs[STAT_BLOB] + hs[STAT_BLOB + 1]; st.blob_tiles_large = hs[STAT_BLOB + 1]; st.blob_tiles_refused = hs[STAT_BLOB + 2]; st.blob_nodes = hs[STAT_BLOB + 3]; st.blob_tris = hs[STAT_BLOB + 4];
    st.tile_rays = hs[STAT_TILE_RAYS]; st.tile_rays_handed_on = hs[STAT_CONT_RAYS];
    for (int k = 0; k < 6; k++) st.tile_diag[k] = hs[STAT_TILE_DIAG + k];
  }
  st.bvh_node_bytes = c->cfg.variant == 1 ? sizeof(Bvh4Node) : c->cfg.variant == 2 ? sizeof(WideNodeQ) : sizeof(BvhNodeQ); st.bvh_tri_bytes = sizeof(TriPacket);
  for (auto& sp : c->spans) {
    float ms = 0.f;
    if (hipEventElapsedTime(&ms, sp.a, sp.b) != hipSuccess) continue;
    switch (sp.cat) {
      case CAT_RAYGEN: st.ms_raygen += ms; break;
      case CAT_TRACE: st.ms_trace_closest += ms; st.launches_trace_closest++; break;
      case CAT_SHADE: st.ms_shade += ms; break;
      case CAT_SHADOW: st.ms_trace_shadow += ms; break;
      case CAT_RESOLVE: st.ms_resolve += ms; break;
      case CAT_FRAME: st.ms_frame += ms; break;
      case CAT_TAIL: st.ms_tail += ms; break;
    }
    if (sp.cat != CAT_FRAME) st.launches_total++;
  }
  if (c->timed_frames > 1) {
    const float k = 1.0f / (float)c->timed_frames;
    st.ms_raygen *= k; st.ms_trace_closest *= k; st.ms_shade *= k; st.ms_trace_shadow *= k; st.ms_resolve *= k; st.ms_frame *= k; st.ms_tail *= k;
    st.launches_trace_closest /= c->timed_frames; st.launches_total /= c->timed_frames;
  }
  st.timed_frames = c->timed_frames;
  st.tail_faults = c->tail_faults;
  st.frames_rerendered = c->frame_rerendered ? 1u : 0u;
  c->ev_used = 0; c->spans.clear(); c->timed_frames = 0;
  c->last = st;
  c->frame_pending = false;
  return RT_OK;
}

}

extern "C" {

int rt_abi_version(void) { return 7; }

static void size_traversal_grids(Scene* S) {
  const int per_cu = S->members.size() >= 3 ? 3 : 5;
  for (rt_ctx* m : S->members)
    if (!m->grid_user_set) m->cfg.trace_blocks = m->n_cu * per_cu;
}

static int create_context(rt_ctx** out_ctx, int device_id, rt_ctx* parent) {
  if (!out_ctx) return fail(nullptr, RT_ERR_INVALID_ARGUMENT, "out_ctx is NULL");
  *out_ctx = nullptr;
  int n = 0;
  hipError_t e = hipGetDeviceCount(&n);
  if (e != hipSuccess || n == 0)
    return fail(nullptr, RT_ERR_NO_DEVICE, "no HIP device available (librt_mi355x has no CPU fallback)");
  if (device_id < 0 || device_id >= n) return fail(nullptr, RT_ERR_INVALID_ARGUMENT, "device_id out of range");
  HIP_TRY(nullptr, hipSetDevice(device_id));
  hipDeviceProp_t prop;
  HIP_TRY(nullptr, hipGetDeviceProperties(&prop, device_id));
  if (std::string(prop.gcnArchName).find("gfx950") == std::string::npos)
    return fail(nullptr, RT_ERR_NO_DEVICE, std::string("device is ") + prop.gcnArchName + ", this library contains gfx950 code only");
  int slot = 0;
  if (parent) {
    while (slot < MAX_SLOTS && (parent->scene->slot_mask >> slot & 1u)) slot++;
    if (slot == MAX_SLOTS) return fail(nullptr, RT_ERR_INVALID_ARGUMENT, "a scene holds at most " + std::to_string(MAX_SLOTS) + " frame slots");
  }
  rt_ctx* c = new rt_ctx();
  c->device = device_id;
  c->n_cu = prop.multiProcessorCount;
  c->info = std::string("gfx950 ") + prop.name + " CUs=" + std::to_string(prop.multiProcessorCount);
  if (hipStreamCreateWithFlags(&c->stream, hipStreamNonBlocking) != hipSuccess) { delete c; return fail(nullptr, RT_ERR_DEVICE, "hipStreamCreate failed"); }
  c->cfg.trace_blocks = c->n_cu * 4;
  c->cfg.shade_blocks = c->n_cu * 8;
  c->cfg.rays_per_lane = 4; c->cfg.min_blocks = c->n_cu;
  c->cfg.variant = 0;
  c->cfg.packet = 0; c->cfg.packet_blocks = c->n_cu * 8;
  if (const char* env = getenv("RT_PACKET")) c->cfg.packet = alt_kernels_built() ? std::max(0, std::min(2, atoi(env))) : 0;
  if (const char* env = getenv("RT_PACKET_BLOCKS_PER_CU")) { const int v = atoi(env); if (v > 0 && v <= 16) c->cfg.packet_blocks = c->n_cu * v; }
  c->tail_resident_per_cu = tail_blocks_per_cu();
  live_slots_add(device_id, 1);
  c->tail_blocks = tail_grid(c->n_cu, c->tail_resident_per_cu, live_slots_on(device_id));
  if (const char* env = getenv("RT_BLAS_BUILDER")) c->blas_builder = atoi(env) ? 1 : 0;
  if (const char* env = getenv("RT_TAIL_MIN_BLOCKS")) c->tail_min_blocks = std::max(1, atoi(env));
  if (getenv("RT_TAIL_FULL_GRID")) c->tail_full_grid = true;
  if (const char* env = getenv("RT_TRACE_VARIANT")) { const int v = atoi(env); c->cfg.variant = (v >= 0 && v <= 2 && alt_kernels_built()) ? v : 0; }
  if (const char* env = getenv("RT_TRACE_BLOCKS_PER_CU")) { int v = atoi(env); if (v > 0 && v <= 8) c->cfg.trace_blocks = c->n_cu * v; }
  if (parent) {
    c->scene = parent->scene;
    c->cfg = parent->cfg; c->blas_builder = parent->blas_builder; c->tail_mode = parent->tail_mode; c->tail_min_blocks = parent->tail_min_blocks; c->tail_full_grid = parent->tail_full_grid; c->primary_cover = parent->primary_cover; c->jitter_table = parent->jitter_table; c->tile_blobs = parent->tile_blobs; c->pixel_beams = parent->pixel_beams; c->camera_records = parent->camera_records; c->dead_shadow_rays = parent->dead_shadow_rays; c->shadow_beams = parent->shadow_beams; c->entry_points = parent->entry_points; c->shadow_entry = parent->shadow_entry; c->entry_max_instances = parent->entry_max_instances; c->light_tiles = parent->light_tiles; c->out_rgba8 = parent->out_rgba8; c->out_bgra = parent->out_bgra;
  } else {
    c->scene = new Scene();
    c->scene->device = device_id;
  }
  c->slot = slot;
  c->scene->slot_mask |= 1u << slot;
  c->scene->members.push_back(c);
  if (getenv("RT_TRACE_BLOCKS_PER_CU")) c->grid_user_set = true;
  if (parent) c->grid_user_set = parent->grid_user_set;
  size_traversal_grids(c->scene);
  *out_ctx = c;
  return RT_OK;
}
// ... 400 lines not shown
    { int q = quiesce_scene(c); if (q) return q; }
    Scene* S = c->scene;
    const int before = c->cfg.variant;
    for (rt_ctx* m : S->members) m->cfg.variant = value;
    bool relink = (value == 2 && before != 2 && S->blas_linked);
    if (value != 0) {
      for (size_t mi = 0; mi < S->meshes.size(); mi++) {
        Mesh& m = S->meshes[mi];
        if (!m.built || !((value == 1 && m.gpu_built) || m.refitted)) continue;
        { int r = sync_host_verts(c, m); if (r) return r; }
        m.refitted = false; m.poisoned = false;
        build_blas(S->h_verts.data() + m.range.first_float, S->h_idx.data() + m.range.first_index, m.range.prim_count, m.bvh, m.tris);
        collapse_bvh4(m.bvh, true, false, m.bvh4);
        m.bounds = m.bvh.bounds; m.gpu_built = false; relink = true;
      }
    }
    if (relink) {
      S->blas_linked = false;
      for (rt_ctx* m : S->members) {
        if (!m->tlas_valid) continue;
        int r;
        if (m->inst_source == INST_DEVICE) {
          m->tlas_valid = false;
          r = set_instances_device(m, m->tgpu.d_rec, m->n_inst, 0, nullptr);
        } else {
          std::vector<rt_instance> keep = m->h_inst;
          m->tlas_valid = false;
          r = rt_set_instances(m, keep.data(), (int)keep.size(), 0);
        }
        if (r) { if (m != c) c->error = m->error; return r; }
      }
    }
    return RT_OK;
  }
  if (k == "closest_blocks_per_cu" || k == "shadow_blocks_per_cu") {
    if (value < -1 || value > 8) return fail(c, RT_ERR_INVALID_ARGUMENT, k + " must be -1 (automatic), 0 (the persistent grid) or 1..8");
    (k[0] == 'c' ? c->closest_blocks_per_cu : c->shadow_blocks_per_cu) = value; return RT_OK;
  }
  if (k == "trace_blocks_per_cu") {
    if (value < 1 || value > 8) return fail(c, RT_ERR_INVALID_ARGUMENT, "trace_blocks_per_cu must be 1..8");
    { int q = quiesce(c); if (q) return q; }
    c->cfg.trace_blocks = c->n_cu * value; c->grid_user_set = true; return RT_OK;
  }
  if (k == "output_rgba8") {
    if (value != 0 && value != 1) return fail(c, RT_ERR_INVALID_ARGUMENT, "output_rgba8 must be 0 or 1");
    if (c->async_pending) return fail(c, RT_ERR_NOT_READY, "output_rgba8 cannot change while a frame is pending");
    c->out_rgba8 = value != 0; c->out_bgra = false; return RT_OK;
  }
  if (k == "output_bgra8") {
    if (value != 0 && value != 1) return fail(c, RT_ERR_INVALID_ARGUMENT, "output_bgra8 must be 0 or 1");
    if (c->async_pending) return fail(c, RT_ERR_NOT_READY, "output_bgra8 cannot change while a frame is pending");
    c->out_rgba8 = value != 0; c->out_bgra = value != 0; return RT_OK;
  }
  if (k == "primary_cover") { c->primary_cover = value != 0; return RT_OK; }
  if (k == "jitter_table") { c->jitter_table = value != 0; return RT_OK; }
  if (k == "tile_blobs") {
    if (value != 0 && !alt_kernels_built()) return fail(c, RT_ERR_INVALID_ARGUMENT, "tile_blobs is not in the product library (measured slower): build librt_mi355x_alt.so with `make alt` and load it (RT_LIB_VARIANT=alt)");
    c->tile_blobs = value != 0; return RT_OK;
  }
  if (k == "pixel_beams") { c->pixel_beams = value != 0; return RT_OK; }
  if (k == "fused_shade") { c->fused_shade = value != 0; return RT_OK; }
  if (k == "camera_records") { c->camera_records = value != 0; return RT_OK; }
  if (k == "dead_shadow_rays") { c->dead_shadow_rays = value != 0; return RT_OK; }
  if (k == "shadow_beams") {
    if (value != 0 && !alt_kernels_built()) return fail(c, RT_ERR_INVALID_ARGUMENT, "shadow_beams is not in the product library (measured slower): build librt_mi355x_alt.so with `make alt` and load it (RT_LIB_VARIANT=alt)");
    c->shadow_beams = value != 0; return RT_OK;
  }

  if (k == "entry_points") { c->entry_points = value != 0; return RT_OK; }
  if (k == "packet_trace") {
    if (value < 0 || value > 2) return fail(c, RT_ERR_INVALID_ARGUMENT, "packet_trace must be 0, 1 or 2");
    if (value != 0 && !alt_kernels_built()) return fail(c, RT_ERR_INVALID_ARGUMENT, "packet_trace is not in the product library (measured slower): build librt_mi355x_alt.so with `make alt` and load it (RT_LIB_VARIANT=alt)");
    c->cfg.packet = value; return RT_OK;
  }
  if (k == "packet_blocks_per_cu") { if (value < 1 || value > 16) return fail(c, RT_ERR_INVALID_ARGUMENT, "packet_blocks_per_cu must be 1..16"); c->cfg.packet_blocks = c->n_cu * value; return RT_OK; }
  if (k == "shadow_entry") { if (value < 0 || value > 2) return fail(c, RT_ERR_INVALID_ARGUMENT, "shadow_entry must be 0, 1 or 2"); if (value != c->shadow_entry) { c->light_built = false; c->light_seen_valid = false; } c->shadow_entry = value; return RT_OK; }
  if (k == "entry_max_instances") { if (value < 1 || value >= (int)ENTRY_NO_INST) return fail(c, RT_ERR_INVALID_ARGUMENT, "entry_max_instances out of range"); c->entry_max_instances = value; return RT_OK; }
  if (k == "light_tiles") {
    if (value < 8 || value > 512) return fail(c, RT_ERR_INVALID_ARGUMENT, "light_tiles must be 8..512");
    { int q = quiesce(c); if (q) return q; }
    c->light_tiles = value; c->light_built = false; return RT_OK;
  }
  if (k == "tail_kernel") { if (value < 0 || value > 2) return fail(c, RT_ERR_INVALID_ARGUMENT, "tail_kernel must be 0 (off), 1 (auto) or 2 (always)"); c->tail_mode = value; return RT_OK; }
  if (k == "debug_force_tail_fault") { c->debug_force_tail_fault = value != 0; if (value == 2) c->tail_disabled = false; return RT_OK; }
  if (k == "blas_builder") { if (value != 0 && value != 1) return fail(c, RT_ERR_INVALID_ARGUMENT, "blas_builder must be 0 (host SAH) or 1 (device)"); for (rt_ctx* m : c->scene->members) m->blas_builder = value; return RT_OK; }
  if (k == "trace_rays_per_lane") { if (value < 1 || value > 64) return fail(c, RT_ERR_INVALID_ARGUMENT, "trace_rays_per_lane must be 1..64"); c->cfg.rays_per_lane = value; return RT_OK; }
  if (k == "trace_min_blocks") { if (value < 8) return fail(c, RT_ERR_INVALID_ARGUMENT, "trace_min_blocks must be >= 8"); c->cfg.min_blocks = value; return RT_OK; }
  if (k == "shade_blocks_per_cu") { if (value < 1 || value > 16) return fail(c, RT_ERR_INVALID_ARGUMENT, "shade_blocks_per_cu must be 1..16"); c->cfg.shade_blocks = c->n_cu * value; return RT_OK; }
  return fail(c, RT_ERR_INVALID_ARGUMENT, "unknown parameter " + k);
}

int rt_debug_check_builders(const float* verts6, size_t n_floats, const uint32_t* idx, size_t n_idx, uint64_t* out) {
  if (!verts6 || !idx || !out || n_idx % 3 != 0) return RT_ERR_INVALID_ARGUMENT;
  const uint32_t n = (uint32_t)(n_idx / 3);
  for (size_t k = 0; k < n_idx; k++) if ((size_t)idx[k] * 6 + 5 >= n_floats) return RT_ERR_INVALID_ARGUMENT;
  BuiltBvh bvh; std::vector<TriPacket> tris; Bvh4 b4; std::vector<BvhNodeQ> q; float q_lo[3], q_scale[3];
  build_blas(verts6, idx, n, bvh, tris);
  collapse_bvh4(bvh, true, false, b4);
  quantize_bvh2(bvh, q, q_lo, q_scale);
  uint64_t violations = 0, reached = 0, max_leaf = 0;
  std::vector<uint8_t> seen(n, 0);
  auto tri_box = [&](uint32_t leaf_pos, Aabb& b) {
    const TriPacket& t = tris[leaf_pos];
    for (int k = 0; k < 3; k++) {
      float a = t.v0[k], c1 = t.v0[k] + t.e1[k], c2 = t.v0[k] + t.e2[k];
      b.lo[k] = std::min(a, std::min(c1, c2)); b.hi[k] = std::max(a, std::max(c1, c2));
    }
  };
  struct Item { int32_t ref; Aabb box; int depth; };
  std::vector<Item> stack;
  auto child_box = [&](const BvhNode& nd, int which) { Aabb b; if (which == 0) { b.lo[0] = nd.a[0]; b.hi[0] = nd.a[1]; b.lo[1] = nd.a[2]; b.hi[1] = nd.a[3]; b.lo[2] = nd.c[0]; b.hi[2] = nd.c[1]; }
                                                        else { b.lo[0] = nd.b[0]; b.hi[0] = nd.b[1]; b.lo[1] = nd.b[2]; b.hi[1] = nd.b[3]; b.lo[2] = nd.c[2]; b.hi[2] = nd.c[3]; } return b; };
  Aabb all; for (int k = 0; k < 3; k++) { all.lo[k] = -3e38f; all.hi[k] = 3e38f; }
  stack.push_back({0, all, 0});
  int depth = 0;
  while (!stack.empty()) {
    Item it = stack.back(); stack.pop_back();
    depth = std::max(depth, it.depth);
    if (it.ref >= 0) {
      if ((size_t)it.ref >= bvh.nodes.size()) { violations++; continue; }
      const BvhNode& nd = bvh.nodes[it.ref]; const BvhNodeQ& nq = q[it.ref];
      for (int w = 0; w < 2; w++) {
        Aabb cb = child_box(nd, w);
        const int32_t ref = w ? nd.child1 : nd.child0;
        if (cb.lo[0] > 1e37f) continue;
        for (int k = 0; k < 3; k++) {
          if (cb.lo[k] < it.box.lo[k] - 1e-4f || cb.hi[k] > it.box.hi[k] + 1e-4f) violations++;
          const uint32_t wq = nq.w[(w ? 3 : 0) + k];
          const double qlo = (double)q_lo[k] + (double)(wq & 0xFFFFu) * q_scale[k], qhi = (double)q_lo[k] + (double)(wq >> 16) * q_scale[k];
          if (qlo > cb.lo[k] || qhi < cb.hi[k]) violations++;
        }
        if ((w ? nq.child1 : nq.child0) != ref) violations++;
        stack.push_back({ref, cb, it.depth + 1});
      }
    } else {
      const uint32_t r = (uint32_t)(~it.ref), first = r >> 3, count = (r & 7u) + 1u;
      max_leaf = std::max<uint64_t>(max_leaf, count);
      for (uint32_t k = 0; k < count; k++) {
        if (first + k >= n) { violations++; continue; }
        const uint32_t prim = tris[first + k].prim;
        if (prim >= n || seen[prim]) violations++; else { seen[prim] = 1; reached++; }
        Aabb tb; tri_box(first + k, tb);
        for (int a = 0; a < 3; a++) if (tb.lo[a] < it.box.lo[a] - 1e-4f || tb.hi[a] > it.box.hi[a] + 1e-4f) violations++;
      }
    }
  }
  if (reached != n) violations++;
  std::vector<uint8_t> seen4(n, 0); uint64_t reached4 = 0;
  std::vector<int32_t> st4; if (!b4.nodes.empty()) st4.push_back(0);
  while (!st4.empty()) {
    int32_t ref = st4.back(); st4.pop_back();
    if (ref >= 0) { for (int k = 0; k < 4; k++) { int32_t c = b4.nodes[ref].c[k].ref; if (c != 0x7FFFFFFF) st4.push_back(c); } }
    else { const uint32_t r = (uint32_t)(~ref), first = r >> 3, count = (r & 7u) + 1u; for (uint32_t k = 0; k < count && first + k < n; k++) { uint32_t p = tris[first + k].prim; if (p < n && !seen4[p]) { seen4[p] = 1; reached4++; } else violations++; } }
  }
  if (reached4 != n) violations++;
  out[0] = bvh.nodes.size(); out[1] = bvh.leaves; out[2] = (uint64_t)depth; out[3] = max_leaf; out[4] = b4.nodes.size(); out[5] = (uint64_t)b4.stack_need;
  out[6] = violations; out[7] = reached;
  return violations ? RT_ERR_INVALID_ARGUMENT : RT_OK;
}

int rt_debug_sizing(int n_cu, int resident_per_cu, int trace_blocks, uint32_t ovf_stride, uint64_t* out) {
  if (!out || n_cu <= 0 || trace_blocks <= 0) return RT_ERR_INVALID_ARGUMENT;
  const int g = tail_grid(n_cu, resident_per_cu, 0);
  out[0] = (uint64_t)g; out[1] = (uint64_t)ovf_elems(trace_blocks, g, ovf_stride);
  return RT_OK;
}

int rt_set_timing(rt_ctx* c, int enabled) { if (!c) return RT_ERR_INVALID_ARGUMENT; c->timing = enabled == 2 ? 2 : (enabled != 0); return RT_OK; }

int rt_trace_shard(rt_ctx* c, int W, int H, int band_rows, int shard, int n_shards, void* d_out, size_t out_capacity_bytes, void* hip_stream) {
  if (!c) return RT_ERR_INVALID_ARGUMENT;
  if (W <= 0 || H <= 0 || band_rows <= 0 || n_shards <= 0 || shard < 0 || shard >= n_shards || !d_out)
    return fail(c, RT_ERR_INVALID_ARGUMENT, "bad rt_trace_shard arguments");
  if (!c->have_uni) return fail(c, RT_ERR_NOT_READY, "rt_set_uniforms has not been called");
  if (c->async_pending) return fail(c, RT_ERR_NOT_READY, "a frame submitted with rt_trace_async is pending: call rt_trace_wait first");
  HIP_TRY(c, hipSetDevice(c->device));
  int r = ready_to_trace(c); if (r) return r;
  const int rows = rt_shard_rows(H, band_rows, shard, n_shards);
  if ((size_t)rows * W * (c->out_rgba8 ? 4 : 16) > out_capacity_bytes) return fail(c, RT_ERR_INVALID_ARGUMENT, "output buffer too small for this shard");
  hipStream_t s = hip_stream ? (hipStream_t)hip_stream : c->stream;
  if (c->frame_pending && c->frame_stream != s) { int q = collect_stats(c); if (q) return q; }
  return enqueue_frame(c, W, H, band_rows, shard, n_shards, (float4*)d_out, s);
}

int rt_trace_shard_batch(rt_ctx* c, int W, int H, int band_rows, int shard, int n_shards, void* d_out, size_t frame_stride_bytes, size_t out_capacity_bytes, void* hip_stream) {
  if (!c) return RT_ERR_INVALID_ARGUMENT;
  if (W <= 0 || H <= 0 || band_rows <= 0 || n_shards <= 0 || shard < 0 || shard >= n_shards || !d_out)
    return fail(c, RT_ERR_INVALID_ARGUMENT, "bad rt_trace_shard_batch arguments");
  if (!c->have_uni) return fail(c, RT_ERR_NOT_READY, "rt_set_batch has not been called");
  if (c->async_pending) return fail(c, RT_ERR_NOT_READY, "a frame submitted with rt_trace_async is pending: call rt_trace_wait first");
  HIP_TRY(c, hipSetDevice(c->device));
  int r = ready_to_trace(c, true); if (r) return r;
  const int rows = rt_shard_rows(H, band_rows, shard, n_shards);
  const size_t px_bytes = c->out_rgba8 ? 4 : 16, shard_bytes = (size_t)rows * W * px_bytes;
  if (frame_stride_bytes == 0) frame_stride_bytes = shard_bytes;
  if (frame_stride_bytes < shard_bytes || frame_stride_bytes % px_bytes != 0 || frame_stride_bytes / px_bytes > 0xFFFFFFFFull)
    return fail(c, RT_ERR_INVALID_ARGUMENT, "frame_stride_bytes must be 0 (compact) or a whole number of pixels >= one shard");
  if (frame_stride_bytes * (size_t)(c->batch_k - 1) + shard_bytes > out_capacity_bytes) return fail(c, RT_ERR_INVALID_ARGUMENT, "output buffer too small for the shards of this batch");
  hipStream_t s = hip_stream ? (hipStream_t)hip_stream : c->stream;
  if (c->frame_pending && c->frame_stream != s) { int q = collect_stats(c); if (q) return q; }
  c->batch_out_stride = (uint32_t)(frame_stride_bytes / px_bytes);
  r = enqueue_frame(c, W, H, band_rows, shard, n_shards, (float4*)d_out, s);
  c->batch_out_stride = 0;
  return r;
}

int rt_assemble_shards(rt_ctx* c, const void* d_gathered, int n_shards, size_t shard_stride_bytes, int W, int H, int band_rows,
                       void* d_frame, size_t frame_capacity_bytes, void* hip_stream) {
  if (!c) return RT_ERR_INVALID_ARGUMENT;
  const size_t bpp = c->out_rgba8 ? 4 : 16;
  if (!d_gathered || !d_frame || n_shards <= 0 || W <= 0 || H <= 0 || band_rows <= 0 || shard_stride_bytes % bpp != 0)
    return fail(c, RT_ERR_INVALID_ARGUMENT, "bad rt_assemble_shards arguments");
  if ((size_t)W * H * bpp > frame_capacity_bytes) return fail(c, RT_ERR_INVALID_ARGUMENT, "frame buffer too small");
  for (int s = 0; s < n_shards; s++)
    if ((size_t)rt_shard_rows(H, band_rows, s, n_shards) * W * bpp > shard_stride_bytes) return fail(c, RT_ERR_INVALID_ARGUMENT, "shard stride smaller than a shard");
  HIP_TRY(c, hipSetDevice(c->device));
  launch_assemble(d_gathered, d_frame, W, H, band_rows, n_shards, shard_stride_bytes / bpp, c->out_rgba8, hip_stream ? (hipStream_t)hip_stream : c->stream);
  HIP_TRY(c, hipGetLastError());
  return RT_OK;
}

int rt_synchronize(rt_ctx* c) {
  if (!c) return RT_ERR_INVALID_ARGUMENT;
  HIP_TRY(c, hipSetDevice(c->device));
  if (c->frame_pending) return collect_stats(c);
  HIP_TRY(c, hipStreamSynchronize(c->stream));
  return RT_OK;
}

int rt_get_stats(rt_ctx* c, rt_stats* st) {
  if (!c || !st) return RT_ERR_INVALID_ARGUMENT;
  int r = collect_stats(c); if (r) return r;
  *st = c->last;
  return RT_OK;
}

static int trace_host(rt_ctx* c, int W, int H, float* out, rt_stats* stats, bool counting) {
  if (!c) return RT_ERR_INVALID_ARGUMENT;
  if (W <= 0 || H <= 0 || !out) return fail(c, RT_ERR_INVALID_ARGUMENT, "bad rt_trace arguments");
  HIP_TRY(c, hipSetDevice(c->device));
  { int q = quiesce(c); if (q) return q; }
  const size_t px = (size_t)W * H;
  if (px > c->out_capacity) {
// ... 419 lines not shown
  return enqueue_query(c, hip_stream ? (hipStream_t)hip_stream : c->stream, c->cfg, Walk::Sweep, n, d_sweeps8, false, false, nullptr, cull_mask, d_hits, d_attr);
}

int rt_sweep_spheres(rt_ctx* c, size_t n, const float* sweeps8, uint32_t cull_mask, rt_hit* out, int counting, rt_stats* stats) {
  if (!c) return RT_ERR_INVALID_ARGUMENT;
  const char* const name = "rt_sweep_spheres";
  if ((!sweeps8 || !out) && n) return fail(c, RT_ERR_INVALID_ARGUMENT, std::string(name) + ": null sweep/hit pointers");
  if (n >= 0xFFFFFF00ull) return fail(c, RT_ERR_INVALID_ARGUMENT, std::string(name) + ": too many sweeps for one call");
  if (cull_mask > 0xFFu) return fail(c, RT_ERR_INVALID_ARGUMENT, std::string(name) + ": cull_mask is above 0xFF");
  if (c->cfg.variant != 0) return fail(c, RT_ERR_INVALID_ARGUMENT, std::string(name) + " needs trace_variant 0");
  HIP_TRY(c, hipSetDevice(c->device));
  { int q = quiesce(c); if (q) return q; }
  int r = ready_to_trace(c); if (r) return r;
  if (stats) memset(stats, 0, sizeof(*stats));
  if (n == 0) return RT_OK;
  const size_t sweep_bytes = n * 8 * sizeof(float);
  char* d_buf = nullptr;
  hipEvent_t e0 = nullptr, e1 = nullptr;
  struct Guard {
    char*& buf; hipEvent_t &a, &b;
    ~Guard() { if (buf) hipFree(buf); if (a) hipEventDestroy(a); if (b) hipEventDestroy(b); }
  } guard{d_buf, e0, e1};
  HIP_TRY(c, hipMalloc((void**)&d_buf, sweep_bytes + n * sizeof(HitRec)));
  HitRec* const d_h = (HitRec*)(d_buf + sweep_bytes);
  HIP_TRY(c, hipMemcpy(d_buf, sweeps8, sweep_bytes, hipMemcpyHostToDevice));
  HIP_TRY(c, hipEventCreate(&e0)); HIP_TRY(c, hipEventCreate(&e1));
  r = enqueue_query(c, c->stream, c->cfg, Walk::Sweep, n, d_buf, false, counting != 0, nullptr, cull_mask, d_h, nullptr, e0, e1); if (r) return r;
  HIP_TRY(c, hipStreamSynchronize(c->stream));
  HIP_TRY(c, hipMemcpy(out, d_h, n * sizeof(HitRec), hipMemcpyDeviceToHost));
  if (stats) {
    if (counting) {
      uint32_t cnt[CNT_TAILS];
      HIP_TRY(c, hipMemcpy(cnt, c->d_q_counters, sizeof(cnt), hipMemcpyDeviceToHost));
      memcpy(&stats->node_visits, &cnt[CNT_NODE_VISITS], 8);
      memcpy(&stats->tri_tests, &cnt[CNT_TRI_TESTS], 8);
    }
    float ms = 0.f; hipEventElapsedTime(&ms, e0, e1);
    stats->ms_trace_closest = ms;
    stats->bvh_node_bytes = sizeof(BvhNodeQ); stats->bvh_tri_bytes = sizeof(TriPacket);
  }
  return RT_OK;
}

int rt_shade_rays_device(rt_ctx* c, size_t n_points, uint32_t n_samples, const void* d_rays8, void* d_sample_rgba, void* d_point_rgba, void* hip_stream) {
  if (!c) return RT_ERR_INVALID_ARGUMENT;
  constexpr size_t MAX_RAYS = (size_t)1 << 25;
  if (n_samples == 0) return fail(c, RT_ERR_INVALID_ARGUMENT, "rt_shade_rays_device: n_samples must be >= 1");
  if (!d_sample_rgba && !d_point_rgba) return fail(c, RT_ERR_INVALID_ARGUMENT, "rt_shade_rays_device: d_sample_rgba and d_point_rgba are both NULL");
  if (n_points > MAX_RAYS || (uint64_t)n_points * n_samples > MAX_RAYS)
    return fail(c, RT_ERR_INVALID_ARGUMENT, "rt_shade_rays_device: at most 2^25 rays (n_points * n_samples) per call");
  const size_t n = n_points * n_samples;
  if (n && !d_rays8) return fail(c, RT_ERR_INVALID_ARGUMENT, "rt_shade_rays_device: d_rays8 is NULL");
  if (((uintptr_t)d_rays8 | (uintptr_t)d_sample_rgba | (uintptr_t)d_point_rgba) & 15u)
    return fail(c, RT_ERR_INVALID_ARGUMENT, "rt_shade_rays_device: rays and outputs must be 16-byte aligned");
  if (c->cfg.variant != 0) return fail(c, RT_ERR_INVALID_ARGUMENT, "rt_shade_rays_device needs trace_variant 0");
  if (c->uni.max_bounce_count + 2 > (uint32_t)CNT_MAX_BOUNCES) return fail(c, RT_ERR_INVALID_ARGUMENT, "maxBounceCount too large (the frame's limit)");
  HIP_TRY(c, hipSetDevice(c->device));
  if (n) {
    const void* ptrs[3] = {d_rays8, d_sample_rgba, d_point_rgba};
    for (const void* p : ptrs) {
      if (!p) continue;
      hipPointerAttribute_t at{};
      const bool ok = hipPointerGetAttributes(&at, p) == hipSuccess && at.type == hipMemoryTypeDevice && at.device == c->device;
      (void)hipGetLastError();
      if (!ok) return fail(c, RT_ERR_INVALID_ARGUMENT, "rt_shade_rays_device: rays and outputs must be device memory of the context's GPU (" + std::to_string(c->device) + ")");
    }
  }
  if (!c->have_uni) return fail(c, RT_ERR_NOT_READY, "rt_set_uniforms has not been called");
  int r = ready_to_trace(c); if (r) return r;
  if (n == 0) return RT_OK;
  hipStream_t s = hip_stream ? (hipStream_t)hip_stream : c->stream;
  const size_t shard_cap = std::max<size_t>(256, ((ray_ingest_block_count((uint32_t)n) + N_SHARDS - 1) / N_SHARDS) * 256);
  const size_t capacity = shard_cap * N_SHARDS;
  const size_t colors = d_sample_rgba ? 0 : n;
  if (capacity > c->shade_capacity || colors > c->shade_colors) {
    { int q = wait_queries(c, c); if (q) return q; }
    const size_t cap = std::max(capacity, c->shade_capacity), col = std::max(colors, c->shade_colors);
    c->shade_capacity = 0; c->shade_colors = 0;
    r = alloc_queues(c, c->shade, cap, cap, col); if (r) return r;
    c->shade_capacity = cap; c->shade_colors = col;
  }
  r = query_workspace(c, s); if (r) return r;
  FrameDev f{};
  for (int k = 0; k < 2; k++) { f.ray_o[k] = c->shade.ray_o[k]; f.ray_d[k] = c->shade.ray_d[k]; }
  f.hit_a = c->shade.hit_a; f.hit_inst = c->shade.hit_inst;
  f.sh_o = c->shade.sh_o; f.sh_d = c->shade.sh_d; f.sh_c = c->shade.sh_c; f.sh_e = c->shade.sh_e;
  f.sample_color = d_sample_rgba ? (float4*)d_sample_rgba : c->shade.sample_color;
  f.counters = c->d_q_counters; f.ovf_stack = c->d_q_ovf;
  f.shard_cap = (uint32_t)shard_cap;
  f.width = (int)n_points; f.height = 1; f.rows = 1; f.band_rows = 1; f.shard = 0; f.n_shards = 1;
  f.batch_k = 1;
  f.far_possible = 1;
  f.settle_dead_shadow_rays = c->dead_shadow_rays;
  LaunchCfg cfg = c->cfg;
  cfg.packet = 0; cfg.far = 1;
  const SceneDev sc = scene_dev(c);
  const UniformsDev u = c->uni;
  const BatchTab bt{};
  HIP_TRY(c, hipMemsetAsync(c->d_q_counters, 0, CNT_WORDS * sizeof(uint32_t), s));
  launch_ray_ingest(sc, f, (const float4*)d_rays8, (uint32_t)n, s);
  for (uint32_t b = 0; b <= u.max_bounce_count; b++) {
    launch_trace_closest(sc, f, (int)b, false, cfg, s);
    launch_shade(sc, f, u, bt, (int)b, cfg, s);
  }
  launch_trace_shadow(sc, f, false, cfg, s);
  if (d_point_rgba) launch_resolve_points(f.sample_color, (float4*)d_point_rgba, (uint32_t)n_points, n_samples, s);
  return query_done(c, s);
}

}
```

vulkan_raytracing_amd/csrc/rt_device.h:

```cpp
#pragma once
#include <stdint.h>

namespace rt {

struct alignas(16) BvhNode {
  float a[4];
  float b[4];
  float c[4];
  int32_t child0, child1;
  int32_t pad0, pad1;
};
static_assert(sizeof(BvhNode) == 64, "BvhNode must be 64 bytes");

struct alignas(16) BvhNodeQ {
  uint32_t w[6];
  int32_t child0, child1;
};
static_assert(sizeof(BvhNodeQ) == 32, "BvhNodeQ must be 32 bytes");

struct alignas(16) WideNodeQ {
  uint32_t x[4], y[4], z[4];
  int32_t ref[4];
};
static_assert(sizeof(WideNodeQ) == 64, "WideNodeQ must be 64 bytes");
// ... 22 lines not shown
struct alignas(16) InstanceDev {
  float w2o[12];
  float o2w[12];
  int32_t blas_root;
  uint32_t mask;
  int32_t custom_index;
  uint32_t first_float;
  uint32_t first_index;
  int32_t blas_root4;
  float q_lo[3];
  float q_scale[3];
  uint32_t type;
  uint32_t cover_first, cover_count;
  uint32_t pad;
};
static_assert(sizeof(InstanceDev) == 160, "InstanceDev must be 160 bytes");

struct UniformsDev {
  float position[4], right[4], up[4], forward[4];
  float light_position[3];
  float light_intensity;
  uint32_t max_bounce_count, samples_per_pixel, center_object_type, orbiting_object_type;
  uint32_t orbiting_object_primitive_offset, orbiting_object_vertex_offset;
};
static_assert(sizeof(UniformsDev) == 104, "UniformsDev must be 104 bytes");

struct HitRec { float t, u, v; int32_t prim, inst; };

struct MaterialDev {
  float ka[3]; float ns;
  float kd[3]; float ni;
  float ks[3]; uint32_t type;
};
static_assert(sizeof(MaterialDev) == 48, "MaterialDev must be 48 bytes");
constexpr uint32_t INST_FLAG_FACING_CULL_DISABLE = 0x1u, INST_FLAG_FLIP_FACING = 0x2u, INST_FLAG_FORCE_OPAQUE = 0x4u, INST_FLAG_FORCE_NO_OPAQUE = 0x8u;
constexpr uint32_t instance_mask_word(uint32_t custom_index_and_mask, uint32_t sbt_offset_and_flags) {
  return (custom_index_and_mask >> 24) | (((sbt_offset_and_flags >> 24) & 0xFu) << 8);
}
constexpr uint32_t QF_OPAQUE = 0x1u, QF_NO_OPAQUE = 0x2u, QF_TERMINATE = 0x4u, QF_CULL_BACK = 0x10u, QF_CULL_FRONT = 0x20u, QF_CULL_OPAQUE = 0x40u,
                   QF_CULL_NO_OPAQUE = 0x80u, QF_SKIP_TRIANGLES = 0x100u, QF_FLAGS = 0x3FFu;
constexpr uint32_t QF_CULL_NEG = 0x400u, QF_CULL_POS = 0x800u;

constexpr uint32_t TYPE_BY_OBJECT_INDEX = 0xFFFFFFFFu;
constexpr uint32_t TYPE_BY_INSTANCE = 0xFFFFFFFFu;
constexpr uint32_t MATERIAL_NONE = 0xFFFFFFFFu;

constexpr int COVER_TARGET_BOXES = 1024;
constexpr int COVER_MAX_TILES = 4096;
constexpr int ENTRY_WORDS = 6;
constexpr uint32_t ENTRY_EMPTY = 0xFFFFFFFFu;
constexpr uint32_t ENTRY_NO_INST = 0xFFFFFFu;
constexpr uint32_t ENTRY_FROM_ROOT = 0x7FFFFFFFu;
constexpr uint32_t ENTRY_REVERSE = 0x80000000u;
struct alignas(16) EntryRec { int32_t w[2 + ENTRY_WORDS]; };
static_assert(sizeof(EntryRec) == 32, "EntryRec must be 32 bytes");
constexpr int ENTRY_VIEWS = 7;
constexpr int BATCH_MAX = 8;
constexpr int MAX_VIEWS = 8;
constexpr int LIGHT_TILES_DEFAULT = 256;
constexpr int BLOB_CLASSES = 3;
constexpr int BLOB_CAP_NODES[BLOB_CLASSES] = {256, 384, 768};
constexpr int BLOB_CAP_TRIS[BLOB_CLASSES] = {170, 256, 512};
constexpr int BLOB_MAX_NODES = BLOB_CAP_NODES[BLOB_CLASSES - 1], BLOB_MAX_TRIS = BLOB_CAP_TRIS[BLOB_CLASSES - 1];
constexpr int BLOB_REST_AT = 64;
constexpr int BLOB_NODES_AT = 128;
constexpr int BLOB_TRIS_AT = BLOB_NODES_AT + BLOB_MAX_NODES * 32;
constexpr int BLOB_SLOT_BYTES = BLOB_TRIS_AT + BLOB_MAX_TRIS * 48;
constexpr int BLOB_MAX_ROOTS = 7;
constexpr int BLOB_MAX_REST = 4;
constexpr uint32_t BLOB_LINK_LEAF = 0x8000u, BLOB_LINK_DONE = 0xFFFFu;
constexpr uint32_t BLOB_NONE = 0xFFFFFFFFu;
constexpr int TILE_STACK = 22;
constexpr uint32_t CONT_FLAG = 0x80000000u;
constexpr int N_SHARDS = 8;
constexpr int CNT_STRIDE = 32;
constexpr int CNT_MAX_BOUNCES = 72;
constexpr int Q_SHADOW = CNT_MAX_BOUNCES;
constexpr int Q_TILE_RAYS = CNT_MAX_BOUNCES + 1;
constexpr int HIT_DEAD = -2;
constexpr int Q_BLOB = CNT_MAX_BOUNCES + 2;
constexpr int Q_BLOB_LIST = CNT_MAX_BOUNCES + 3;
constexpr int Q_DEAD = Q_BLOB_LIST + BLOB_CLASSES;
constexpr int Q_SHADOW0 = Q_DEAD + 1;
constexpr int N_QUEUES = Q_SHADOW0 + 1;
constexpr int TAIL_BLOCKS = 64;
constexpr int MAX_TAILS_IN_FLIGHT = 16;
constexpr uint32_t TAIL_MAX_RAYS = 16384;
enum : int {
  CNT_NODE_VISITS = 0,
  CNT_TRI_TESTS = 2,
  CNT_NODE_VISITS_SH = 4,
  CNT_TRI_TESTS_SH = 6,
  CNT_DIAG = 8,
  CNT_DIAG_SH = 16,
  CNT_BARRIER = 24,
  CNT_FAULT = 25,
  CNT_TILE_DIAG = 32,
  CNT_BLOB_STATS = 26,
  CNT_TAILS = 48
};
enum StatSlot : int {
  STAT_QUEUE0 = 0,
  STAT_SECONDARY = 1,
  STAT_SHADOW = 2,
  STAT_QUEUE1 = 3,
  STAT_FAULT = 4,
  STAT_NODE_VISITS = 5, STAT_TRI_TESTS = 6, STAT_NODE_VISITS_SH = 7, STAT_TRI_TESTS_SH = 8,
  STAT_DIAG = 9,
  STAT_FAULT_TOTAL = 15,
  STAT_BLOB = 16,
  STAT_TILE_RAYS = 21,
  STAT_CONT_RAYS = 22,
  STAT_TILE_DIAG = 23,
  STAT_SHADOW_UNTRACED = 29,
  STAT_WORDS = 32
};
constexpr int CNT_WORKS = CNT_TAILS + N_QUEUES * N_SHARDS * CNT_STRIDE;
constexpr int CNT_WORDS = CNT_WORKS + N_QUEUES * N_SHARDS * CNT_STRIDE;
constexpr inline int cnt_tail(int queue, int shard) { return CNT_TAILS + (queue * N_SHARDS + shard) * CNT_STRIDE; }
constexpr inline int cnt_work(int queue, int shard) { return CNT_WORKS + (queue * N_SHARDS + shard) * CNT_STRIDE; }

constexpr uint32_t SID_DEAD = 0xFFFFFFFFu;
#ifndef RT_LDS_INSTANCES
#define RT_LDS_INSTANCES 32
#endif
constexpr int LDS_INSTANCES = RT_LDS_INSTANCES;
constexpr int STACK4_LDS = 64;
constexpr int STACK_LDS = 24;
constexpr int STACK_OVF = 40;
constexpr int BLAS_MAX_DEPTH = 40;

}
```

vulkan_raytracing_amd/csrc/rt_kernels.h:

```cpp
#pragma once
#include <hip/hip_runtime.h>
#include <stdint.h>

#include "rt_device.h"

namespace rt {

struct SceneDev {
  const BvhNodeQ* blas_nodes;
  int tlas_root;
  int tlas_nodes;
  int tlas_stride;
  uint32_t batch_samples;
  const float4* tris;
  float tlas_q_lo[3], tlas_q_scale[3];
  const WideNodeQ* wide_nodes;
  const Bvh4Node* nodes4;
  int tlas_root4;
  const InstanceDev* inst;
  const float* verts;
  const uint32_t* idx;
  const uchar4* sky;
  int n_inst;
  int sky_w, sky_h;
  uint32_t ovf_stride;
  const MaterialDev* materials;
  const uint32_t* prim_material;
  int n_materials;
  const float* cover_boxes;
};

struct FrameDev {
  float4* ray_o[2];
  float4* ray_d[2];
  float4* hit_a;
  int32_t* hit_inst;
  float4* sh_o;
  float4* sh_d;
  float4* sh_c;
  float4* sample_color;
  uint32_t* counters;
  uint32_t* counters_next;
  int32_t* ovf_stack;
  unsigned long long* stats_out;
  uint32_t* fault_total;
  uint32_t* hint;
  float4* out;
  int out_rgba8;
  uint32_t shard_cap;
  int width, height;
  int rows;
  int band_rows, shard, n_shards;
  const uint32_t* cover;
  uint32_t* cover_next;
  uint32_t cover_words;
  int cover_tiles_x;
  EntryRec* entry;
  const EntryRec* light_entry;
  uint32_t* sh_e;
  int light_tiles;
  int far_possible;
  int settle_dead_shadow_rays;
  const float2* jitter;
  int batch_k;
  uint32_t out_frame_stride;
  uint32_t cover_view_words;
  uint32_t* tile_blob;
  char* blob_arena;
  uint32_t blob_slots;
  uint4* blob_list;
  int pixel_runs;
  uint32_t shadow_runs;
  uint32_t sh_base;
};

struct CoverArgs {
  float cam[3];
  float inv[9];
  float kf;
  float apex_radius;
  int width, height, tiles_x, tiles_y;
  int n_inst;
  uint32_t mask_offset;
  int inst_base;
};
struct CoverViews { CoverArgs v[MAX_VIEWS]; int n; };

struct EntryArgs {
  float cam[3];
  float inv[9];
  float basis[9];
  float kf;
  float apex_radius;
  int width, height;
  int tiles_x, tile_rows;
  int band_rows, shard, n_shards;
  EntryRec* records;
  const uint32_t* cover;
  int cover_tiles_x;
  int tlas_root_offset;
};
struct EntryViews { EntryArgs v[MAX_VIEWS]; int n; };

struct BatchTab {
  float position[BATCH_MAX][4], right[BATCH_MAX][4], up[BATCH_MAX][4], forward[BATCH_MAX][4];
  float light[BATCH_MAX][4];
};

struct LaunchCfg {
  int trace_blocks;
  int shade_blocks;
  int rays_per_lane;
  int min_blocks;
  int variant;
  int far;
  int packet;
  int packet_blocks;
};

size_t raygen_block_count(int width, int rows, uint32_t spp, int batch_k);
void launch_raygen(const SceneDev& sc, const FrameDev& f, const UniformsDev& u, const BatchTab& bt, hipStream_t s);
size_t jitter_table_elems(int width, int rows, uint32_t spp);
void launch_jitter_table(const FrameDev& f, uint32_t spp, float2* table, hipStream_t s);
void launch_trace_closest(const SceneDev& sc, const FrameDev& f, int bounce, bool counting, const LaunchCfg& cfg, hipStream_t s);
void launch_beam_shade(const SceneDev& sc, const FrameDev& f, const UniformsDev& u, const LaunchCfg& cfg, hipStream_t s);
void launch_entry(const SceneDev& sc, const EntryViews& a, hipStream_t s);
void launch_blob(const SceneDev& sc, const EntryArgs& e, const FrameDev& f, bool counting, hipStream_t s);
void launch_tile(const SceneDev& sc, const FrameDev& f, const UniformsDev& u, bool counting, hipStream_t s);
void launch_tail(const SceneDev& sc, const FrameDev& f, const UniformsDev& u, const BatchTab& bt, int first_bounce, bool counting, const LaunchCfg& cfg, int tail_blocks, hipStream_t s);
void launch_shade(const SceneDev& sc, const FrameDev& f, const UniformsDev& u, const BatchTab& bt, int bounce, const LaunchCfg& cfg, hipStream_t s);
void launch_beam_shadow(const SceneDev& sc, const FrameDev& f, const UniformsDev& u, bool counting, const LaunchCfg& cfg, hipStream_t s);
void launch_trace_shadow(const SceneDev& sc, const FrameDev& f, bool counting, const LaunchCfg& cfg, hipStream_t s);
void launch_resolve(const FrameDev& f, const UniformsDev& u, hipStream_t s);
void launch_cover(const SceneDev& sc, const CoverViews& a, uint32_t max_boxes_per_instance, uint32_t* mask_block, hipStream_t s);
void launch_query(const SceneDev& sc, const float4* rays, HitRec* out, uint32_t n, int32_t* ovf_stack, uint32_t* counters, bool any_hit,
                  bool counting, const LaunchCfg& cfg, hipStream_t s);
void launch_hit_attr(const SceneDev& sc, const HitRec* hits, float4* attr, uint32_t n, hipStream_t s);
void launch_query_flags(const SceneDev& sc, const float4* rays, const uint32_t* words, uint32_t query_word, HitRec* out, uint32_t n,
                        int32_t* ovf_stack, uint32_t* counters, const LaunchCfg& cfg, hipStream_t s);
void launch_hit_kind(const SceneDev& sc, const float4* rays, const HitRec* hits, float4* attr, uint32_t n, hipStream_t s);
void launch_query_hits(const SceneDev& sc, const float4* rays, const uint32_t* words, uint32_t query_word, uint32_t n, uint32_t k, HitRec* hits,
                       float4* attr, uint32_t* counts, int32_t* ovf_stack, uint32_t* counters, const LaunchCfg& cfg, hipStream_t s);
void launch_closest_scale(const SceneDev& sc, float* inst_scale, hipStream_t s);
void launch_closest_point(const SceneDev& sc, const float4* points, uint32_t cull_mask, const float* inst_scale, HitRec* hits, uint32_t n, int32_t* ovf_stack,
                          uint32_t* counters, bool counting, const LaunchCfg& cfg, hipStream_t s);
void launch_closest_side(const SceneDev& sc, const float4* points, const HitRec* hits, float4* attr, uint32_t n, hipStream_t s);
void launch_overlap_boxes(const SceneDev& sc, const float4* boxes, uint32_t cull_mask, const float* inst_scale, bool any, uint32_t k, void* ids, uint32_t* counts,
                          uint32_t n, int32_t* ovf_stack, uint32_t* counters, bool counting, const LaunchCfg& cfg, hipStream_t s);
void launch_sweep_spheres(const SceneDev& sc, const float4* sweeps, uint32_t cull_mask, const float* inst_scale, HitRec* hits, uint32_t n, int32_t* ovf_stack,
                          uint32_t* counters, bool counting, const LaunchCfg& cfg, hipStream_t s);
void launch_sweep_side(const SceneDev& sc, const float4* sweeps, const HitRec* hits, float4* attr, uint32_t n, hipStream_t s);
uint32_t ray_ingest_block_count(uint32_t n);
void launch_ray_ingest(const SceneDev& sc, const FrameDev& f, const float4* rays, uint32_t n, hipStream_t s);
void launch_resolve_points(const float4* sample_color, float4* out, uint32_t n_points, uint32_t n_samples, hipStream_t s);

void launch_assemble(const void* gathered, void* out, int width, int height, int band_rows, int n_shards, size_t shard_stride_px, bool rgba8, hipStream_t s);
int trace_threads_per_block();
bool alt_kernels_built();
int tail_blocks_per_cu();
size_t ovf_elems(int trace_blocks, int tail_blocks, uint32_t stride);
int tail_grid(int n_cu, int resident_blocks_per_cu, int live_slots);

}
```

Before: 34810.

## Overlap tail bounces with shadow tracing in a single split-role kernel

Adds a k_tail_shadow kernel. A subset of blocks runs the persistent tail bounce loop, with its grid barrier scoped to those blocks, while the remaining blocks trace shadow rays from the main queue at the same time. Shadow rays produced during tail bounces go to a separate tail queue filled from the top of the buffer, and the tail blocks drain it afterwards. The aim is to fill the GPU left idle by the small tail grid, at the cost of a larger overflow-stack allocation, lower occupancy from the merged kernel, and a risk of the two queues colliding in a shared buffer.

```diff
diff --git a/include/rt_api.h b/include/rt_api.h
--- a/include/rt_api.h
+++ b/include/rt_api.h
@@ -192,6 +192,7 @@
 
 int rt_debug_check_builders(const float* verts6, size_t n_floats, const uint32_t* idx, size_t n_idx, uint64_t* out8);
 int rt_debug_sizing(int n_cu, int resident_per_cu, int trace_blocks, uint32_t ovf_stride, uint64_t* out2);
+int rt_debug_sizing_tail_shadow(int n_cu, int resident_per_cu, int trace_blocks, uint32_t ovf_stride, uint64_t* out3);
 
 const char* rt_last_error(const rt_ctx* ctx);
 const char* rt_device_info(const rt_ctx* ctx);
diff --git a/vulkan_raytracing_amd/api.py b/vulkan_raytracing_amd/api.py
--- a/vulkan_raytracing_amd/api.py
+++ b/vulkan_raytracing_amd/api.py
@@ -58,7 +58,7 @@
 
 EXPORTS = ["rt_create", "rt_create_frame_slot", "rt_destroy", "rt_upload_geometry", "rt_build_blas", "rt_set_instances", "rt_set_instances_device", "rt_refit_blas_device", "rt_set_materials", "rt_set_instance_types", "rt_set_uniforms", "rt_set_skybox",
            "rt_trace", "rt_trace_async", "rt_trace_wait", "rt_trace_shard", "rt_set_batch", "rt_trace_shard_batch", "rt_assemble_shards", "rt_shard_rows", "rt_synchronize", "rt_get_stats", "rt_set_timing", "rt_intersect",
-           "rt_trace_counting", "rt_intersect_device", "rt_intersect_device_flags", "rt_intersect_device_hits", "rt_closest_point_device", "rt_closest_point", "rt_overlap_boxes_device", "rt_overlap_boxes", "rt_sweep_spheres_device", "rt_sweep_spheres", "rt_shade_rays_device", "rt_set_param", "rt_debug_check_builders", "rt_debug_sizing", "rt_last_error", "rt_device_info", "rt_abi_version"]
+           "rt_trace_counting", "rt_intersect_device", "rt_intersect_device_flags", "rt_intersect_device_hits", "rt_closest_point_device", "rt_closest_point", "rt_overlap_boxes_device", "rt_overlap_boxes", "rt_sweep_spheres_device", "rt_sweep_spheres", "rt_shade_rays_device", "rt_set_param", "rt_debug_check_builders", "rt_debug_sizing", "rt_debug_sizing_tail_shadow", "rt_last_error", "rt_device_info", "rt_abi_version"]
 
 _LIBS = {}
 
@@ -95,6 +95,8 @@
         L.rt_set_param.argtypes = [vp, C.c_char_p, C.c_int]
         L.rt_debug_check_builders.argtypes = [vp, C.c_size_t, vp, C.c_size_t, vp]
         L.rt_debug_sizing.argtypes = [C.c_int, C.c_int, C.c_int, C.c_uint32, vp]
+        if hasattr(L, "rt_debug_sizing_tail_shadow"):
+            L.rt_debug_sizing_tail_shadow.argtypes = [C.c_int, C.c_int, C.c_int, C.c_uint32, vp]
         L.rt_intersect.argtypes = [vp, C.c_size_t, vp, C.c_int, vp, C.c_int, C.POINTER(RtStats)]
         L.rt_intersect_device.argtypes = [vp, C.c_size_t, vp, C.c_int, vp, vp, vp]
         L.rt_intersect_device_flags.argtypes = [vp, C.c_size_t, vp, vp, C.c_uint32, C.c_uint32, vp, vp, vp]
diff --git a/vulkan_raytracing_amd/csrc/kernels.hip b/vulkan_raytracing_amd/csrc/kernels.hip
--- a/vulkan_raytracing_amd/csrc/kernels.hip
+++ b/vulkan_raytracing_amd/csrc/kernels.hip
@@ -847,16 +847,24 @@
 #define PH_END(k)
 #endif
 
-template <int MODE, bool ANY, bool COUNT, bool WIDE, bool ENTRY = false, bool FAR = true, bool CONT = false>
-__device__ __forceinline__ void trace_body(const TraceArgs& a) {
+__shared__ int s_trace_stack[4][STACK2_LDS + 1][64];
+__shared__ float4 s_trace_rays[4][2][64];
+__shared__ float4 s_trace_out[4][64];
+__shared__ int2 s_trace_outq[4][64];
+__shared__ uint32_t s_trace_ent4[4][64], s_trace_ent1[1][64];
+__shared__ float4 s_trace_inst[LDS_INSTANCES ? LDS_INSTANCES : 1][5];
+
+template <int MODE, bool ANY, bool COUNT, bool WIDE, bool ENTRY = false, bool FAR = true, bool CONT = false, bool REVQ = false>
+__device__ __forceinline__ void trace_body(const TraceArgs& a, const uint32_t vblock = blockIdx.x, const bool rev = false) {
   constexpr bool RAYS8 = MODE == MODE_QUERY || MODE == MODE_QUERY_FLAGS;
   constexpr bool QF = MODE == MODE_QUERY_FLAGS;
-  __shared__ int s_stack[4][STACK2_LDS + 1][64];
-  __shared__ float4 s_rays[4][2][64];
-  __shared__ float4 s_out[4][64];
-  __shared__ int2 s_outq[4][64];
-  __shared__ uint32_t s_ent[((ENTRY && MODE == MODE_SHADOW) || QF) ? 4 : 1][64];
-  __shared__ float4 s_inst[LDS_INSTANCES ? LDS_INSTANCES : 1][5];
+  const bool down = REVQ && rev;
+  auto& s_stack = s_trace_stack;
+  auto& s_rays = s_trace_rays;
+  auto& s_out = s_trace_out;
+  auto& s_outq = s_trace_outq;
+  auto& s_ent = *[] { if constexpr ((ENTRY && MODE == MODE_SHADOW) || QF) return &s_trace_ent4; else return &s_trace_ent1; }();
+  auto& s_inst = s_trace_inst;
   {
     uint32_t total = 0;
 #pragma unroll
@@ -864,7 +872,7 @@
     uint32_t want = (total + 256u * a.rays_per_lane - 1u) / (256u * a.rays_per_lane);
     want = (want + (N_SHARDS - 1)) & ~(uint32_t)(N_SHARDS - 1);
     if (want < a.min_blocks) want = a.min_blocks;
-    if (blockIdx.x >= want) return;
+    if (vblock >= want) return;
   }
   const int n_lds_inst = a.sc.n_inst < LDS_INSTANCES ? a.sc.n_inst : LDS_INSTANCES;
   if ((int)threadIdx.x < n_lds_inst) {
@@ -893,7 +901,7 @@
       uint32_t off = 0;
       if (lane == 0 && size) off = atomicAdd(a.work + shard * CNT_STRIDE, 64u);
       off = (uint32_t)__builtin_amdgcn_readfirstlane((int)off);
-      if (size && off < size) { pf_base = shard * a.shard_cap + off; pf_count = (size - off) < 64u ? (size - off) : 64u; break; }
+      if (size && off < size) { pf_base = shard * a.shard_cap + off; if constexpr (REVQ) { if (down) pf_base = shard * a.shard_cap + (a.shard_cap - 1u - off); } pf_count = (size - off) < 64u ? (size - off) : 64u; break; }
       shard = (shard + 1u) & (N_SHARDS - 1); tried++;
     }
     if (lane < pf_count) {
@@ -905,9 +913,15 @@
           pf_e = ((a.query_word | w) & QF_FLAGS) | (a.query_word & w & 0xFF000000u);
         }
       } else {
-        pf_o = ld_stream(&a.ray_o[pf_base + lane]); pf_d = ld_stream(&a.ray_d[pf_base + lane]);
-      }
-      if (ENTRY && MODE == MODE_SHADOW) pf_e = (uint32_t)ld_stream(reinterpret_cast<const int*>(a.sh_e) + pf_base + lane);
+        if constexpr (REVQ) {
+          const uint32_t r = down ? pf_base - lane : pf_base + lane;
+          pf_o = ld_stream(&a.ray_o[r]); pf_d = ld_stream(&a.ray_d[r]);
+        } else {
+          pf_o = ld_stream(&a.ray_o[pf_base + lane]); pf_d = ld_stream(&a.ray_d[pf_base + lane]);
+        }
+      }
+      if constexpr (REVQ) { if (ENTRY && MODE == MODE_SHADOW) pf_e = (uint32_t)ld_stream(reinterpret_cast<const int*>(a.sh_e) + (down ? pf_base - lane : pf_base + lane)); }
+      else if (ENTRY && MODE == MODE_SHADOW) pf_e = (uint32_t)ld_stream(reinterpret_cast<const int*>(a.sh_e) + pf_base + lane);
     }
   };
   auto promote = [&]() {
@@ -994,6 +1008,7 @@
         if (need && rank < avail) {
           const uint32_t ci = chunk_pos + rank;
           q = chunk_base + ci;
+          if constexpr (REVQ) { if (down) q = chunk_base - ci; }
           const float4 ro = s_rays[wave][0][ci], rd = s_rays[wave][1][ci];
           if (RAYS8) { tmin_ray = ro.w; tmax = rd.w; }
           else { tmax = ro.w; sid = __float_as_uint(rd.w); }
@@ -1474,9 +1489,12 @@
     const uint64_t m_sh = __ballot(push_shadow);
     if (lane == 0 && m_sh != 0ull) __hip_atomic_fetch_add(f.counters + cnt_tail(Q_SHADOW0, (int)shard), (uint32_t)__builtin_popcountll(m_sh), __ATOMIC_RELAXED, __HIP_MEMORY_SCOPE_AGENT);
   } else {
-    const uint32_t slot_s = wave_alloc(push_shadow, f.counters + cnt_tail(Q_SHADOW, (int)shard));
+    bool to_tail = false;
+    if constexpr (!REG) to_tail = (uint32_t)bounce >= f.shadow_split;
+    const uint32_t slot_s = wave_alloc(push_shadow, f.counters + cnt_tail(to_tail ? Q_SHADOW_TAIL : Q_SHADOW, (int)shard));
     if (push_shadow) {
-      const uint32_t v = f.sh_base + shard * f.shard_cap + slot_s;
+      const uint32_t v = to_tail ? shard * f.shard_cap + (f.shard_cap - 1u - slot_s)
+                                 : f.sh_base + shard * f.shard_cap + slot_s;
       st_stream(&f.sh_o[v], make_float4(no.x, no.y, no.z, sh_tmax));
       st_stream(&f.sh_d[v], make_float4(nd.x, nd.y, nd.z, __uint_as_float(sid)));
       st_stream(&f.sh_c[v], make_float4(sh_c.x, sh_c.y, sh_c.z, sh_w));
@@ -1486,7 +1504,7 @@
 }
 
 template <bool TILE = false, bool BATCH = false, bool RUNS = false>
-__device__ __forceinline__ void shade_body(const ShadeArgs& a, const int bounce) {
+__device__ __forceinline__ void shade_body(const ShadeArgs& a, const int bounce, const uint32_t n_blocks = gridDim.x) {
   const FrameDev& f = a.f;
   const UniformsDev& U = a.u;
   const uint32_t lane = threadIdx.x & 63u, wave = threadIdx.x >> 6;
@@ -1503,7 +1521,7 @@
     } else cnt[t] = ld_cursor(f.counters + cnt_tail(bounce, t));
     maxb = max(maxb, (cnt[t] + 63u) >> 6);
   }
-  const uint32_t n_waves = gridDim.x * 4u;
+  const uint32_t n_waves = n_blocks * 4u;
   for (uint32_t g = blockIdx.x * 4u + wave; g < maxb * N_SHARDS; g += n_waves) {
     const uint32_t shard = g & (N_SHARDS - 1), base = (g >> 3) << 6;
     uint32_t n = 0;
@@ -1529,12 +1547,12 @@
   uint32_t* fault;
 };
 
-__device__ __forceinline__ void grid_barrier(uint32_t* bar, uint32_t* fault, uint32_t& phase) {
+__device__ __forceinline__ void grid_barrier(uint32_t* bar, uint32_t* fault, uint32_t& phase, const uint32_t n_blocks = gridDim.x) {
   __syncthreads();
   phase++;
   if (threadIdx.x == 0) {
     __threadfence();
-    const uint32_t target = phase * gridDim.x;
+    const uint32_t target = phase * n_blocks;
     __hip_atomic_fetch_add(bar, 1u, __ATOMIC_RELAXED, __HIP_MEMORY_SCOPE_AGENT);
     uint32_t spins = 0;
     while (__hip_atomic_load(bar, __ATOMIC_RELAXED, __HIP_MEMORY_SCOPE_AGENT) < target) {
@@ -1567,6 +1585,59 @@
     if (ld_cursor(t.fault) != 0u) return;
   }
 }
+
+#ifndef RT_ALT_KERNELS
+struct TailShadowArgs {
+  TailArgs t;
+  uint32_t tail_blocks;
+  uint32_t sh_rays_per_lane, sh_min_blocks;
+};
+#ifndef RT_TAIL_SHADOW_WAVES
+#define RT_TAIL_SHADOW_WAVES 0
+#endif
+template <bool ENTRY>
+__global__ __launch_bounds__(256)
+#if RT_TAIL_SHADOW_WAVES > 0
+__attribute__((amdgpu_waves_per_eu(RT_TAIL_SHADOW_WAVES, RT_TAIL_SHADOW_WAVES)))
+#endif
+void k_tail_shadow(TailShadowArgs ts) {
+  const TailArgs& t = ts.t;
+  const uint32_t tb = ts.tail_blocks;
+  const bool tail_role = blockIdx.x < tb;
+  if (tail_role) {
+    uint32_t phase = 0;
+    const uint32_t max_bounce = t.sh.u.max_bounce_count;
+    for (uint32_t b = t.first_bounce; b <= max_bounce; b++) {
+      uint32_t live = 0;
+#pragma unroll
+      for (int k = 0; k < N_SHARDS; k++) live += ld_cursor(t.tr.counters + cnt_tail((int)b, k));
+      if (live == 0) break;
+      if (ld_cursor(t.fault) != 0u) return;
+      TraceArgs a = t.tr;
+      a.ray_o = t.sh.f.ray_o[b & 1u]; a.ray_d = t.sh.f.ray_d[b & 1u];
+      a.tails = t.tr.counters + cnt_tail((int)b, 0);
+      a.work = t.tr.counters + cnt_work((int)b, 0);
+      trace_body<MODE_CLOSEST, false, false, false>(a, blockIdx.x, false);
+      grid_barrier(t.barrier, t.fault, phase, tb);
+      if (ld_cursor(t.fault) != 0u) return;
+      shade_body<false, false>(t.sh, (int)b, tb);
+      grid_barrier(t.barrier, t.fault, phase, tb);
+      if (ld_cursor(t.fault) != 0u) return;
+    }
+  }
+  TraceArgs a = t.tr;
+  const FrameDev& f = t.sh.f;
+  a.ray_o = f.sh_o; a.ray_d = f.sh_d; a.sh_c = f.sh_c; a.sample_color = f.sample_color;
+  a.entry = ENTRY ? f.light_entry : nullptr; a.sh_e = ENTRY ? f.sh_e : nullptr;
+  const int queue = tail_role ? Q_SHADOW_TAIL : Q_SHADOW;
+  a.tails = t.tr.counters + cnt_tail(queue, 0);
+  a.work = t.tr.counters + cnt_work(queue, 0);
+  if (!tail_role) a.ovf_stack = f.ovf_stack - (size_t)tb * 256u * (size_t)a.sc.ovf_stride;
+  a.rays_per_lane = tail_role ? 1u : ts.sh_rays_per_lane;
+  a.min_blocks = tail_role ? (uint32_t)N_SHARDS : ts.sh_min_blocks;
+  trace_body<MODE_SHADOW, true, false, false, ENTRY, false, false, true>(a, tail_role ? blockIdx.x : blockIdx.x - tb, tail_role);
+}
+#endif
 
 __global__ __launch_bounds__(256) void k_resolve(FrameDev f, UniformsDev u) {
   const uint32_t npx1 = (uint32_t)(f.rows * f.width);
@@ -1615,7 +1686,7 @@
       else if (t >= STAT_BLOB && t < STAT_BLOB + 5) v = ld_cursor(f.counters + CNT_BLOB_STATS + (int)(t - STAT_BLOB));
       else if (t >= STAT_TILE_DIAG && t < STAT_TILE_DIAG + 6) v = cnt64(CNT_TILE_DIAG + 2 * (int)(t - STAT_TILE_DIAG));
       else if (t == STAT_SECONDARY) { for (uint32_t b = 1; b <= u.max_bounce_count && b < (uint32_t)CNT_MAX_BOUNCES; b++) v += s_q[b]; }
-      else if (t == STAT_SHADOW) v = s_q[Q_SHADOW] + s_q[Q_SHADOW0];
+      else if (t == STAT_SHADOW) v = s_q[Q_SHADOW] + s_q[Q_SHADOW0] + s_q[Q_SHADOW_TAIL];
       else if (t == STAT_SHADOW_UNTRACED) { for (int k = 0; k < N_SHARDS; k++) v += ld_cursor(f.counters + cnt_work(Q_DEAD, k)); }
       else if (t == STAT_QUEUE1) v = s_q[1];
       else if (t == STAT_FAULT) v = ld_cursor(f.counters + CNT_FAULT);
@@ -2028,8 +2099,35 @@
   n = min(n, v);
   if (hipOccupancyMaxActiveBlocksPerMultiprocessor(&v, k_tail<true, true>, 256, 0) != hipSuccess) return 0;
   n = min(n, v);
+#else
+  if (hipOccupancyMaxActiveBlocksPerMultiprocessor(&v, k_tail_shadow<true>, 256, 0) != hipSuccess) return 0;
+  n = min(n, v);
+  if (hipOccupancyMaxActiveBlocksPerMultiprocessor(&v, k_tail_shadow<false>, 256, 0) != hipSuccess) return 0;
+  n = min(n, v);
 #endif
   return n;
+}
+
+bool launch_tail_shadow(const SceneDev& sc, const FrameDev& f, const UniformsDev& u, int first_bounce, const LaunchCfg& cfg, int tail_blocks, int32_t* tail_ovf, hipStream_t s) {
+#ifndef RT_ALT_KERNELS
+  TailShadowArgs ts{};
+  TailArgs& t = ts.t;
+  t.tr = make_args(sc, f.counters, first_bounce, f.shard_cap, tail_ovf);
+  t.tr.hit_a = f.hit_a; t.tr.hit_inst = f.hit_inst;
+  t.tr.rays_per_lane = 1u; t.tr.min_blocks = 8u;
+  t.sh = ShadeArgs{sc, f, u, first_bounce, BatchTab{}};
+  t.first_bounce = (uint32_t)first_bounce;
+  t.barrier = f.counters + CNT_BARRIER; t.fault = f.counters + CNT_FAULT;
+  ts.tail_blocks = (uint32_t)tail_blocks;
+  const bool entry = f.light_entry != nullptr && f.sh_e != nullptr;
+  ts.sh_rays_per_lane = (uint32_t)cfg.rays_per_lane; ts.sh_min_blocks = (uint32_t)cfg.min_blocks;
+  const dim3 g((unsigned)(tail_blocks + cfg.trace_blocks)), b(256);
+  if (entry) hipLaunchKernelGGL((k_tail_shadow<true>), g, b, 0, s, ts);
+  else hipLaunchKernelGGL((k_tail_shadow<false>), g, b, 0, s, ts);
+  return true;
+#else
+  return false;
+#endif
 }
 
 void launch_tail(const SceneDev& sc, const FrameDev& f, const UniformsDev& u, const BatchTab& bt, int first_bounce, bool counting, const LaunchCfg& cfg, int tail_blocks, hipStream_t s) {
diff --git a/vulkan_raytracing_amd/csrc/rt_api.cpp b/vulkan_raytracing_amd/csrc/rt_api.cpp
--- a/vulkan_raytracing_amd/csrc/rt_api.cpp
+++ b/vulkan_raytracing_amd/csrc/rt_api.cpp
@@ -63,7 +63,7 @@
 };
 
 struct TimedSpan { int cat; hipEvent_t a, b; };
-enum { CAT_RAYGEN = 0, CAT_TRACE, CAT_SHADE, CAT_SHADOW, CAT_RESOLVE, CAT_FRAME, CAT_TAIL, CAT_N };
+enum { CAT_RAYGEN = 0, CAT_TRACE, CAT_SHADE, CAT_SHADOW, CAT_RESOLVE, CAT_FRAME, CAT_TAIL, CAT_TAIL_SHADOW, CAT_N };
 
 }
 
@@ -154,6 +154,7 @@
   uint32_t ovf_stride = STACK_OVF, ovf_alloc_stride = 0;
   int stack_need = 0;
   int ovf_alloc_blocks = 0;
+  int ovf_alloc_tail = 0;
   char* h_stage[2] = {nullptr, nullptr};
   size_t stage_bytes[2] = {0, 0};
   hipEvent_t ev_upload[2] = {nullptr, nullptr};
@@ -238,6 +239,7 @@
   uint32_t tail_faults = 0;
   uint32_t* d_fault_total = nullptr;
   uint64_t faults_seen = 0;
+  bool tail_overlap = true;
   bool debug_force_tail_fault = false;
   uint32_t last_max_bounce = 0;
   uint64_t last_primary = 0;
@@ -307,6 +309,9 @@
 
 size_t rt::ovf_elems(int trace_blocks, int tail_blocks, uint32_t stride) {
   return (size_t)std::max(trace_blocks, tail_blocks) * 256u * (size_t)stride;
+}
+size_t rt::tail_ovf_elems(int tail_blocks, uint32_t stride) {
+  return (size_t)std::max(tail_blocks, 0) * 256u * (size_t)stride;
 }
 int rt::tail_grid(int n_cu, int resident_blocks_per_cu, int live_slots) {
   const long cap = (long)n_cu * std::max(0, resident_blocks_per_cu) / std::max(MAX_TAILS_IN_FLIGHT, live_slots);
@@ -760,10 +765,10 @@
     memset(c->h_stats, 0, STAT_WORDS * sizeof(unsigned long long));
     HIP_TRY(c, hipHostGetDevicePointer((void**)&c->d_stats, c->h_stats, 0));
   }
-  if (c->d_ovf && (c->ovf_alloc_stride < c->ovf_stride || c->ovf_alloc_blocks < std::max(c->cfg.trace_blocks, c->tail_blocks))) { HIP_TRY(c, hipFree(c->d_ovf)); c->d_ovf = nullptr; }
+  if (c->d_ovf && (c->ovf_alloc_stride < c->ovf_stride || c->ovf_alloc_blocks < std::max(c->cfg.trace_blocks, c->tail_blocks) || c->ovf_alloc_tail < c->tail_blocks)) { HIP_TRY(c, hipFree(c->d_ovf)); c->d_ovf = nullptr; }
   if (!c->d_ovf) {
-    HIP_TRY(c, hipMalloc((void**)&c->d_ovf, ovf_elems(c->cfg.trace_blocks, c->tail_blocks, c->ovf_stride) * sizeof(int32_t)));
-    c->ovf_alloc_stride = c->ovf_stride; c->ovf_alloc_blocks = std::max(c->cfg.trace_blocks, c->tail_blocks);
+    HIP_TRY(c, hipMalloc((void**)&c->d_ovf, (ovf_elems(c->cfg.trace_blocks, c->tail_blocks, c->ovf_stride) + tail_ovf_elems(c->tail_blocks, c->ovf_stride)) * sizeof(int32_t)));
+    c->ovf_alloc_stride = c->ovf_stride; c->ovf_alloc_blocks = std::max(c->cfg.trace_blocks, c->tail_blocks); c->ovf_alloc_tail = c->tail_blocks;
   }
   return RT_OK;
 }
@@ -1035,6 +1040,7 @@
   f.pixel_runs = beam_on ? 64 * (int)std::min<uint32_t>(u.samples_per_pixel, 4u) : 0;
   f.shadow_runs = (beam_on && c->shadow_beams && K == 1 && std::isfinite(u.light_position[0]) && std::isfinite(u.light_position[1]) && std::isfinite(u.light_position[2])) ? 1u : 0u;
   f.sh_base = f.shadow_runs ? (uint32_t)capacity : 0u;
+  f.shadow_split = 0xFFFFFFFFu;
   if (c->jitter_table && rows > 0) { r = jitter_table_for(c, f, u.samples_per_pixel, s, &f.jitter); if (r) return r; }
   if (!c->timing || c->timed_frames >= 64) { c->ev_used = 0; c->spans.clear(); c->timed_frames = 0; }
   if (c->timing) c->timed_frames++;
@@ -1069,17 +1075,30 @@
     else if (tail_ok && c->tail_mode == 1)
       for (uint32_t b = 1; b <= u.max_bounce_count && b < (uint32_t)CNT_MAX_BOUNCES; b++)
         if (((volatile uint32_t*)c->h_hint)[b] <= TAIL_MAX_RAYS) { tail_start = b; break; }
+    int tb = 0;
+    if (tail_start != 0xFFFFFFFFu && tail_start <= u.max_bounce_count) {
+      tb = std::min(c->tail_blocks, tail_grid(c->n_cu, c->tail_resident_per_cu, live_slots_on(c->device)));
+      const uint32_t expect = ((volatile uint32_t*)c->h_hint)[tail_start];
+      if (tb > 0 && c->tail_mode == 1 && expect != 0xFFFFFFFFu && !c->tail_full_grid && c->scene->members.size() >= 3) {
+        long want = ((long)expect + 255) / 256;
+        const long lo = c->tail_min_blocks;
+        if (lo >= N_SHARDS) want = (want + (N_SHARDS - 1)) / N_SHARDS * N_SHARDS;
+        tb = (int)std::min<long>(tb, std::max<long>(lo, want));
+      }
+    }
+    const bool overlap = c->tail_overlap && tb > 0 && K == 1 && !c->counting && c->cfg.variant == 0 && !cfg.packet && !f.shadow_runs && !f.tile_blob &&
+                         cfg.far == 0 && !again && !alt_kernels_built();
+    if (overlap) f.shadow_split = tail_start;
+    bool shadow_done = false;
     const bool fused0 = c->fused_shade && beam_on && c->camera_records && K == 1 && !c->counting && !f.tile_blob && !f.shadow_runs && tail_start != 0u;
     for (uint32_t b = 0; b <= u.max_bounce_count; b++) {
       if (b == tail_start) {
-        int tb = std::min(c->tail_blocks, tail_grid(c->n_cu, c->tail_resident_per_cu, live_slots_on(c->device)));
         if (tb <= 0) { { Span sp(c, CAT_TRACE, s); launch_trace_closest(sc, f, (int)b, c->counting, cfg, s); } { Span sp(c, CAT_SHADE, s); launch_shade(sc, f, u, bt, (int)b, cfg, s); } continue; }
-        const uint32_t expect = ((volatile uint32_t*)c->h_hint)[b];
-        if (c->tail_mode == 1 && expect != 0xFFFFFFFFu && !c->tail_full_grid && c->scene->members.size() >= 3) {
-          long want = ((long)expect + 255) / 256;
-          const long lo = c->tail_min_blocks;
-          if (lo >= N_SHARDS) want = (want + (N_SHARDS - 1)) / N_SHARDS * N_SHARDS;
-          tb = (int)std::min<long>(tb, std::max<long>(lo, want));
+        if (overlap) {
+          LaunchCfg cs = cfg; if (cap_shadow > 0) cs.trace_blocks = std::min(cfg.trace_blocks, c->n_cu * cap_shadow);
+          Span sp(c, CAT_TAIL_SHADOW, s);
+          shadow_done = launch_tail_shadow(sc, f, u, (int)b, cs, tb, c->d_ovf + ovf_elems(c->ovf_alloc_blocks, 0, c->ovf_alloc_stride), s);
+          if (shadow_done) break;
         }
         Span sp(c, CAT_TAIL, s); launch_tail(sc, f, u, bt, (int)b, c->counting, cfg, tb, s);
         break;
@@ -1099,6 +1118,7 @@
         if (live == 0) break;
       }
     }
+    if (!shadow_done)
     { LaunchCfg cs = cfg; if (cap_shadow > 0) cs.trace_blocks = std::min(cfg.trace_blocks, c->n_cu * cap_shadow);
       Span sp(c, CAT_SHADOW, s); launch_beam_shadow(sc, f, u, c->counting, cs, s); launch_trace_shadow(sc, f, c->counting, cs, s); }
     { Span sp(c, CAT_RESOLVE, s); launch_resolve(f, u, s); }
@@ -1164,6 +1184,7 @@
       case CAT_RESOLVE: st.ms_resolve += ms; break;
       case CAT_FRAME: st.ms_frame += ms; break;
       case CAT_TAIL: st.ms_tail += ms; break;
+      case CAT_TAIL_SHADOW: st.ms_trace_shadow += ms; st.ms_tail += ms; break;
     }
     if (sp.cat != CAT_FRAME) st.launches_total++;
   }
@@ -1730,6 +1751,7 @@
     c->light_tiles = value; c->light_built = false; return RT_OK;
   }
   if (k == "tail_kernel") { if (value < 0 || value > 2) return fail(c, RT_ERR_INVALID_ARGUMENT, "tail_kernel must be 0 (off), 1 (auto) or 2 (always)"); c->tail_mode = value; return RT_OK; }
+  if (k == "tail_overlap") { c->tail_overlap = value != 0; return RT_OK; }
   if (k == "debug_force_tail_fault") { c->debug_force_tail_fault = value != 0; if (value == 2) c->tail_disabled = false; return RT_OK; }
   if (k == "blas_builder") { if (value != 0 && value != 1) return fail(c, RT_ERR_INVALID_ARGUMENT, "blas_builder must be 0 (host SAH) or 1 (device)"); for (rt_ctx* m : c->scene->members) m->blas_builder = value; return RT_OK; }
   if (k == "trace_rays_per_lane") { if (value < 1 || value > 64) return fail(c, RT_ERR_INVALID_ARGUMENT, "trace_rays_per_lane must be 1..64"); c->cfg.rays_per_lane = value; return RT_OK; }
@@ -1807,6 +1829,12 @@
   return violations ? RT_ERR_INVALID_ARGUMENT : RT_OK;
 }
 
+int rt_debug_sizing_tail_shadow(int n_cu, int resident_per_cu, int trace_blocks, uint32_t ovf_stride, uint64_t* out) {
+  if (!out) return RT_ERR_INVALID_ARGUMENT;
+  const int g = tail_grid(n_cu, resident_per_cu, 0);
+  out[0] = (uint64_t)g; out[1] = (uint64_t)ovf_elems(trace_blocks, g, ovf_stride); out[2] = (uint64_t)tail_ovf_elems(g, ovf_stride);
+  return RT_OK;
+}
 int rt_debug_sizing(int n_cu, int resident_per_cu, int trace_blocks, uint32_t ovf_stride, uint64_t* out) {
   if (!out || n_cu <= 0 || trace_blocks <= 0) return RT_ERR_INVALID_ARGUMENT;
   const int g = tail_grid(n_cu, resident_per_cu, 0);
@@ -2392,6 +2420,7 @@
   }
   r = query_workspace(c, s); if (r) return r;
   FrameDev f{};
+  f.shadow_split = 0xFFFFFFFFu;
   for (int k = 0; k < 2; k++) { f.ray_o[k] = c->shade.ray_o[k]; f.ray_d[k] = c->shade.ray_d[k]; }
   f.hit_a = c->shade.hit_a; f.hit_inst = c->shade.hit_inst;
   f.sh_o = c->shade.sh_o; f.sh_d = c->shade.sh_d; f.sh_c = c->shade.sh_c; f.sh_e = c->shade.sh_e;
diff --git a/vulkan_raytracing_amd/csrc/rt_device.h b/vulkan_raytracing_amd/csrc/rt_device.h
--- a/vulkan_raytracing_amd/csrc/rt_device.h
+++ b/vulkan_raytracing_amd/csrc/rt_device.h
@@ -128,7 +128,8 @@
 constexpr int Q_BLOB_LIST = CNT_MAX_BOUNCES + 3;
 constexpr int Q_DEAD = Q_BLOB_LIST + BLOB_CLASSES;
 constexpr int Q_SHADOW0 = Q_DEAD + 1;
-constexpr int N_QUEUES = Q_SHADOW0 + 1;
+constexpr int Q_SHADOW_TAIL = Q_SHADOW0 + 1;
+constexpr int N_QUEUES = Q_SHADOW_TAIL + 1;
 constexpr int TAIL_BLOCKS = 64;
 constexpr int MAX_TAILS_IN_FLIGHT = 16;
 constexpr uint32_t TAIL_MAX_RAYS = 16384;
diff --git a/vulkan_raytracing_amd/csrc/rt_kernels.h b/vulkan_raytracing_amd/csrc/rt_kernels.h
--- a/vulkan_raytracing_amd/csrc/rt_kernels.h
+++ b/vulkan_raytracing_amd/csrc/rt_kernels.h
@@ -72,6 +72,7 @@
   int pixel_runs;
   uint32_t shadow_runs;
   uint32_t sh_base;
+  uint32_t shadow_split;
 };
 
 struct CoverArgs {
@@ -128,6 +129,7 @@
 void launch_blob(const SceneDev& sc, const EntryArgs& e, const FrameDev& f, bool counting, hipStream_t s);
 void launch_tile(const SceneDev& sc, const FrameDev& f, const UniformsDev& u, bool counting, hipStream_t s);
 void launch_tail(const SceneDev& sc, const FrameDev& f, const UniformsDev& u, const BatchTab& bt, int first_bounce, bool counting, const LaunchCfg& cfg, int tail_blocks, hipStream_t s);
+bool launch_tail_shadow(const SceneDev& sc, const FrameDev& f, const UniformsDev& u, int first_bounce, const LaunchCfg& cfg, int tail_blocks, int32_t* tail_ovf, hipStream_t s);
 void launch_shade(const SceneDev& sc, const FrameDev& f, const UniformsDev& u, const BatchTab& bt, int bounce, const LaunchCfg& cfg, hipStream_t s);
 void launch_beam_shadow(const SceneDev& sc, const FrameDev& f, const UniformsDev& u, bool counting, const LaunchCfg& cfg, hipStream_t s);
 void launch_trace_shadow(const SceneDev& sc, const FrameDev& f, bool counting, const LaunchCfg& cfg, hipStream_t s);
@@ -159,6 +161,7 @@
 bool alt_kernels_built();
 int tail_blocks_per_cu();
 size_t ovf_elems(int trace_blocks, int tail_blocks, uint32_t stride);
+size_t tail_ovf_elems(int tail_blocks, uint32_t stride);
 int tail_grid(int n_cu, int resident_blocks_per_cu, int live_slots);
 
 }
```

Result: slower. 34350 (-1.3%).
